# nadult/Snail

Measured on AMD Instinct MI355X. Metric: Mrays/sec (primary), higher is better.
Workload: dtype f32

## Files before the change

### snail_amd/csrc/snail_dev.inc

```
namespace SNAIL_DEV_NS {

typedef unsigned long long u64;
typedef unsigned u32x4 __attribute__((ext_vector_type(4)));
typedef const __attribute__((address_space(4))) u32x4 *scalar_ptr;

struct Node {
	float bmin[3], bmax[3];
	unsigned sub;
	int aux;
};

__device__ __forceinline__ float asf(unsigned u) { return __uint_as_float(u); }
__device__ __forceinline__ float asf(int u) { return __int_as_float(u); }

typedef const __attribute__((address_space(4))) char *scalar_bytes;
__device__ __forceinline__ Node loadNode(const uint4 *nodes, int idx) {
	const unsigned off = (unsigned)idx << 5;
	scalar_ptr p = (scalar_ptr)((scalar_bytes)(unsigned long long)nodes + off);
	u32x4 a = p[0], b = p[1];
	Node n;
	n.bmin[0] = asf(a.x); n.bmin[1] = asf(a.y); n.bmin[2] = asf(a.z);
	n.bmax[0] = asf(a.w); n.bmax[1] = asf(b.x); n.bmax[2] = asf(b.y);
	n.sub = b.z; n.aux = (int)b.w;
	return n;
// ... 627 lines not shown
		st.intersects += width;
	}
	const int q = lane - first;
#pragma unroll
	for(int l = 0; l < 4; l++) {
		const int src = (q * LPQ + l / R) * 4;
		const float d = xbar(src, ndist[l % R]);
		const int nt = __builtin_amdgcn_ds_bpermute(src, ntid[l % R]);
		if(inRange && nt >= 0) { Q.dist[l] = d; tid[l] = nt; }
	}
}
template <bool MASK, int M, bool BARY>
__device__ __forceinline__ void leafPerRay(const uint4 *__restrict__ tris, int count, int firstTri, int lane, int first, int last, const float (&org)[3][4],
										   Quad &Q, unsigned mask4, int (&tid)[4], float (&bu)[4], float (&bv)[4], Counters &st) {
	const bool inRange = lane >= first && lane <= last;
	const int width = last - first + 1;
	if(!BARY) {
		const int widthU = __builtin_amdgcn_readfirstlane(width);
		if(widthU <= 32) {
			const int firstU = __builtin_amdgcn_readfirstlane(first);
			if(widthU <= 16) leafPerRayNarrow<1, MASK, M>(tris, __builtin_amdgcn_readfirstlane(count), firstTri, lane, firstU, firstU + widthU - 1, org, Q, mask4, tid, st);
			else leafPerRayNarrow<2, MASK, M>(tris, __builtin_amdgcn_readfirstlane(count), firstTri, lane, firstU, firstU + widthU - 1, org, Q, mask4, tid, st);
			return;
		}
	}
	st.leaves++; st.fetched += (unsigned)count;
	for(int k = 0; k < count; k++) {
		const Tri t = loadTriScalar(tris, firstTri + k);
#pragma unroll
		for(int l = 0; l < 4; l++) {
			const float det = Q.d[0][l] * t.n[0] + Q.d[1][l] * t.n[1] + Q.d[2][l] * t.n[2];
			float tv[3] = {org[0][l] - t.a[0], org[1][l] - t.a[1], org[2][l] - t.a[2]};
			float c0[3] = {t.ba[1] * tv[2] - t.ba[2] * tv[1], t.ba[2] * tv[0] - t.ba[0] * tv[2], t.ba[0] * tv[1] - t.ba[1] * tv[0]};
			float c1[3] = {tv[1] * t.ca[2] - tv[2] * t.ca[1], tv[2] * t.ca[0] - tv[0] * t.ca[2], tv[0] * t.ca[1] - tv[1] * t.ca[0]};
			const float tmul = -(tv[0] * t.n[0] + tv[1] * t.n[1] + tv[2] * t.n[2]);
			const float v = (Q.d[0][l] * c0[0] + Q.d[1][l] * c0[1] + Q.d[2][l] * c0[2]) * t.it0;
			const float u = (Q.d[0][l] * c1[0] + Q.d[1][l] * c1[1] + Q.d[2][l] * c1[2]) * t.it0;
			const float duv = det - u - v;
			const float uvmin = Min3<M>(u, v, duv), uvmax = Max3<M>(u, v, duv);
			bool test = ((uvmax <= 0.0f) | (uvmin >= 0.0f)) & inRange;
			if(MASK) test = test & (((mask4 >> l) & 1u) != 0);
			if(test) {
				const float idet = Inv(det);
				const float dd = idet * tmul;
				if(dd < Q.dist[l] && dd > 0.0f) {
					Q.dist[l] = dd; tid[l] = firstTri + k;
					if(BARY) { bu[l] = u * idet; bv[l] = v * idet; }
				}
			}
		}
		st.intersects += width;
	}
}

template <bool SHARED, bool MASK, bool SHADOW, int M, bool BARY, bool DEEP, bool DISTPOS>
__device__ __forceinline__ void walk(const uint4 *__restrict__ nodes, const uint4 *__restrict__ tris, int size, int lane,
									 const float (&org)[3][4] , Quad &Q, unsigned mask4, int (&tid)[4],
									 float (&bu)[4], float (&bv)[4], float *lds, Counters &st, const int oct = 0) {
	constexpr bool EXACT = M == M_EXACT;
	Interval iv;
	{
		unsigned act4 = lane < size ? 15u : 0u;
		if(SHADOW) {
			act4 = 0;
			if(lane < size)
#pragma unroll
				for(int l = 0; l < 4; l++) act4 |= (Q.dist[l] >= 0.0f ? 1u : 0u) << l;
		} else if(MASK) act4 = lane < size ? (mask4 & 15u) : 0u;
		computeMinMax<EXACT, (MASK || SHADOW)>(Q.d, act4, size, lane, lds, iv.minDir, iv.maxDir);
		if(EXACT) computeMinMax<EXACT, (MASK || SHADOW)>(Q.id, act4, size, lane, lds, iv.minIDir, iv.maxIDir);
		else {
#pragma unroll
			for(int k = 0; k < 3; k++) iv.minIDir[k] = iv.maxIDir[k] = 0.0f;
		}
		if(SHARED) {
#pragma unroll
			for(int k = 0; k < 3; k++) iv.minOrg[k] = iv.maxOrg[k] = org[k][0];
		} else computeMinMax<EXACT, MASK>(org, act4, size, lane, lds, iv.minOrg, iv.maxOrg);
	}

	const int signBits = __builtin_amdgcn_readfirstlane((Q.d[0][0] < 0.0f ? 1 : 0) | (Q.d[1][0] < 0.0f ? 2 : 0) | (Q.d[2][0] < 0.0f ? 4 : 0));
	const int octMask[3] = {-(oct & 1), -((oct >> 1) & 1), -((oct >> 2) & 1)};

	int stkNode = 0, stkFL = 0, stkNode2 = 0, stkFL2 = 0;
	int sp = 0;
	int first = 0, last = size - 1;
	Node n = loadNode(nodes, 0);

	for(;;) {
		st.iters++;
		const bool isLeaf = (n.sub & 0x80000000u) != 0;
		const int axis = n.aux & 0xffff;
		const int firstNode = ((n.aux >> 16) ^ (signBits >> axis)) & 1;
		const int nearIdx = isLeaf ? 0 : (int)n.sub + firstNode;
		const int farIdx = (int)n.sub + (firstNode ^ 1);
		const Node nn = loadNode(nodes, nearIdx);

		auto fastPass = [&](const Node &n) -> u64 {
			float tn[4], tf[4];
			if(M == M_COH) {
				float pn[3], pf[3];
#pragma unroll
				for(int k = 0; k < 3; k++) {
					const int lo = __float_as_int(n.bmin[k]), hi = __float_as_int(n.bmax[k]);
					const int sw = (lo ^ hi) & octMask[k];
					pn[k] = __int_as_float(lo ^ sw); pf[k] = __int_as_float(hi ^ sw);
					if(SHARED) { pn[k] = pn[k] - org[k][0]; pf[k] = pf[k] - org[k][0]; }
				}
#pragma unroll
				for(int l = 0; l < 4; l++) {
					float lo[3], hi[3];
#pragma unroll
					for(int k = 0; k < 3; k++) {
						lo[k] = Q.id[k][l] * (SHARED ? pn[k] : pn[k] - org[k][l]);
						hi[k] = Q.id[k][l] * (SHARED ? pf[k] : pf[k] - org[k][l]);
					}
					tn[l] = vmax3(lo[0], lo[1], lo[2]);
					tf[l] = vmin3(hi[0], hi[1], hi[2]);
				}
			} else {
				float pn[3], pf[3];
#pragma unroll
				for(int k = 0; k < 3; k++) { pn[k] = SHARED ? n.bmin[k] - org[k][0] : n.bmin[k]; pf[k] = SHARED ? n.bmax[k] - org[k][0] : n.bmax[k]; }
#pragma unroll
				for(int l = 0; l < 4; l++) {
					float lo[3], hi[3];
#pragma unroll
					for(int k = 0; k < 3; k++) {
						const float a = Q.id[k][l] * (SHARED ? pn[k] : pn[k] - org[k][l]);
						const float b = Q.id[k][l] * (SHARED ? pf[k] : pf[k] - org[k][l]);
						lo[k] = vmin(a, b); hi[k] = vmax(a, b);
					}
					tn[l] = vmax3(lo[0], lo[1], lo[2]);
					tf[l] = vmin3(hi[0], hi[1], hi[2]);
				}
			}
			if(DISTPOS) {
#pragma unroll
				for(int l = 0; l < 4; l++) { tn[l] = vmax(tn[l], 0.0f); tf[l] = vmin(tf[l], Q.dist[l]); }
				const float slack = vmax3(tf[0] - tn[0], tf[1] - tn[1], vmax(tf[2] - tn[2], tf[3] - tn[3]));
				return __builtin_amdgcn_ballot_w64(slack >= 0.0f);
			} else {
				float sl[4];
#pragma unroll
				for(int l = 0; l < 4; l++) sl[l] = vmin(vmin(tf[l], Q.dist[l]) - tn[l], tf[l]);
				const float slack = vmax3(sl[0], sl[1], vmax(sl[2], sl[3]));
				return __builtin_amdgcn_ballot_w64(slack >= 0.0f);
			}
				};
		u64 passMask = 0;
		if(EXACT) {
			bool anyPass = false;
			if(boxTestInterval(n, iv)) {
				float tmn[3], tmx[3];
				if(SHARED) {
#pragma unroll
					for(int k = 0; k < 3; k++) { tmn[k] = n.bmin[k] - org[k][0]; tmx[k] = n.bmax[k] - org[k][0]; }
				}
#pragma unroll
				for(int l = 0; l < 4; l++) {
					float lmin = 0.0f, lmax = 0.0f;
#pragma unroll
					for(int k = 0; k < 3; k++) {
						float l1 = Q.id[k][l] * (SHARED ? tmn[k] : n.bmin[k] - org[k][l]);
						float l2 = Q.id[k][l] * (SHARED ? tmx[k] : n.bmax[k] - org[k][l]);
						float lo = Min<M_EXACT>(l1, l2), hi = Max<M_EXACT>(l1, l2);
						if(k == 0) { lmin = lo; lmax = hi; }
						else if(SHADOW) { lmin = Max<M_EXACT>(lo, lmin); lmax = Min<M_EXACT>(hi, lmax); }
						else { lmin = Max<M_EXACT>(lmin, lo); lmax = Min<M_EXACT>(lmax, hi); }
					}
					bool pass = SHADOW ? (lmax >= 0.0f && lmin <= Min<M_EXACT>(lmax, Q.dist[l])) : !(lmax < 0.0f || lmin > Min<M_EXACT>(lmax, Q.dist[l]));
					anyPass |= pass;
				}
			}
			passMask = __builtin_amdgcn_ballot_w64(anyPass);
		} else passMask = fastPass(n);
		const u64 alive = passMask & __builtin_amdgcn_ballot_w64((unsigned)(lane - first) <= (unsigned)(last - first));
		if(alive != 0) {
			first = __builtin_ctzll(alive);
			last = 63 - __builtin_clzll(alive);
			if(!isLeaf) {
				const int fl = first | (last << 8);
				if(!DEEP || sp < 64) writeLane2(stkNode, farIdx, stkFL, fl, sp);
				else writeLane2(stkNode2, farIdx, stkFL2, fl, sp - 64);
				sp++;
				n = nn;
				continue;
			}
		const int count = n.aux, firstTri = (int)(n.sub & 0x7fffffffu);
		if(SHARED) {
			if(leafShared<MASK, SHADOW, M, BARY>(tris, count, firstTri, size, lane, first, last, org, Q, mask4, tid, bu, bv, iv, st)) return;
		} else {
			leafPerRay<MASK, M, BARY>(tris, count, firstTri, lane, first, last, org, Q, mask4, tid, bu, bv, st);
		}
		}
		if(sp == 0) break;
		sp--;
		int cur, fl;
		if(!DEEP || sp < 64) { cur = __builtin_amdgcn_readlane(stkNode, sp); fl = __builtin_amdgcn_readlane(stkFL, sp); }
		else { cur = __builtin_amdgcn_readlane(stkNode2, sp - 64); fl = __builtin_amdgcn_readlane(stkFL2, sp - 64); }
		first = fl & 0xff; last = fl >> 8;
		n = loadNode(nodes, cur);
	}
}

#define SNAIL_SLAB_COH(L, NX, FX, NY, FY, NZ, FZ)                                                                                           \
	"v_mul_f32 %[t0], %[ix" L "], %[pnx]\n v_mul_f32 %[t1], %[iy" L "], %[pny]\n v_mul_f32 %[t2], %[iz" L "], %[pnz]\n"                    \
	"v_mul_f32 %[t3], %[ix" L "], %[pfx]\n v_mul_f32 %[t4], %[iy" L "], %[pfy]\n v_mul_f32 %[t5], %[iz" L "], %[pfz]\n"                    \
	"v_max3_f32 %[t0], %[t0], %[t1], %[t2]\n v_min3_f32 %[t3], %[t3], %[t4], %[t5]\n"
#define SNAIL_SLAB_FAST(L, NX, FX, NY, FY, NZ, FZ)                                                                                          \
	"v_mul_f32 %[t0], %[ix" L "], %[pnx]\n v_mul_f32 %[t3], %[ix" L "], %[pfx]\n v_min_f32 %[u0], %[t0], %[t3]\n v_max_f32 %[t3], %[t0], %[t3]\n" \
	"v_mul_f32 %[t1], %[iy" L "], %[pny]\n v_mul_f32 %[t4], %[iy" L "], %[pfy]\n v_min_f32 %[t0], %[t1], %[t4]\n v_max_f32 %[t4], %[t1], %[t4]\n" \
	"v_mul_f32 %[t2], %[iz" L "], %[pnz]\n v_mul_f32 %[t5], %[iz" L "], %[pfz]\n v_min_f32 %[t1], %[t2], %[t5]\n v_max_f32 %[t5], %[t2], %[t5]\n" \
	"v_max3_f32 %[t0], %[u0], %[t0], %[t1]\n v_min3_f32 %[t3], %[t3], %[t4], %[t5]\n"
#define SNAIL_SLAB_COH_R(L, NX, FX, NY, FY, NZ, FZ)                                                                                         \
	"v_mul_f32 %[t0], " NX ", %[ix" L "]\n v_mul_f32 %[t1], " NY ", %[iy" L "]\n v_mul_f32 %[t2], " NZ ", %[iz" L "]\n"                    \
	"v_mul_f32 %[t3], " FX ", %[ix" L "]\n v_mul_f32 %[t4], " FY ", %[iy" L "]\n v_mul_f32 %[t5], " FZ ", %[iz" L "]\n"                    \
	"v_max3_f32 %[t0], %[t0], %[t1], %[t2]\n v_min3_f32 %[t3], %[t3], %[t4], %[t5]\n"
#define SNAIL_SLAB_FAST_R(L, NX, FX, NY, FY, NZ, FZ)                                                                                        \
	"v_mul_f32 %[t0], " NX ", %[ix" L "]\n v_mul_f32 %[t3], " FX ", %[ix" L "]\n v_min_f32 %[u0], %[t0], %[t3]\n v_max_f32 %[t3], %[t0], %[t3]\n" \
	"v_mul_f32 %[t1], " NY ", %[iy" L "]\n v_mul_f32 %[t4], " FY ", %[iy" L "]\n v_min_f32 %[t0], %[t1], %[t4]\n v_max_f32 %[t4], %[t1], %[t4]\n" \
	"v_mul_f32 %[t2], " NZ ", %[iz" L "]\n v_mul_f32 %[t5], " FZ ", %[iz" L "]\n v_min_f32 %[t1], %[t2], %[t5]\n v_max_f32 %[t5], %[t2], %[t5]\n" \
	"v_max3_f32 %[t0], %[u0], %[t0], %[t1]\n v_min3_f32 %[t3], %[t3], %[t4], %[t5]\n"
#define SNAIL_SLABO_COH(L, NX, FX, NY, FY, NZ, FZ)                                                                                          \
	"v_sub_f32 %[t0], " NX ", %[ox" L "]\n v_sub_f32 %[t1], " NY ", %[oy" L "]\n v_sub_f32 %[t2], " NZ ", %[oz" L "]\n"                    \
	"v_sub_f32 %[t3], " FX ", %[ox" L "]\n v_sub_f32 %[t4], " FY ", %[oy" L "]\n v_sub_f32 %[t5], " FZ ", %[oz" L "]\n"                    \
	"v_mul_f32 %[t0], %[ix" L "], %[t0]\n v_mul_f32 %[t1], %[iy" L "], %[t1]\n v_mul_f32 %[t2], %[iz" L "], %[t2]\n"                       \
	"v_mul_f32 %[t3], %[ix" L "], %[t3]\n v_mul_f32 %[t4], %[iy" L "], %[t4]\n v_mul_f32 %[t5], %[iz" L "], %[t5]\n"                       \
	"v_max3_f32 %[t0], %[t0], %[t1], %[t2]\n v_min3_f32 %[t3], %[t3], %[t4], %[t5]\n"
#define SNAIL_SLABO_FAST(L, NX, FX, NY, FY, NZ, FZ)                                                                                         \
	"v_sub_f32 %[t0], " NX ", %[ox" L "]\n v_sub_f32 %[t3], " FX ", %[ox" L "]\n v_mul_f32 %[t0], %[ix" L "], %[t0]\n v_mul_f32 %[t3], %[ix" L "], %[t3]\n" \
	"v_min_f32 %[u0], %[t0], %[t3]\n v_max_f32 %[t3], %[t0], %[t3]\n"                                                                      \
	"v_sub_f32 %[t1], " NY ", %[oy" L "]\n v_sub_f32 %[t4], " FY ", %[oy" L "]\n v_mul_f32 %[t1], %[iy" L "], %[t1]\n v_mul_f32 %[t4], %[iy" L "], %[t4]\n" \
	"v_min_f32 %[t0], %[t1], %[t4]\n v_max_f32 %[t4], %[t1], %[t4]\n"                                                                      \
	"v_sub_f32 %[t2], " NZ ", %[oz" L "]\n v_sub_f32 %[t5], " FZ ", %[oz" L "]\n v_mul_f32 %[t2], %[iz" L "], %[t2]\n v_mul_f32 %[t5], %[iz" L "], %[t5]\n" \
	"v_min_f32 %[t1], %[t2], %[t5]\n v_max_f32 %[t5], %[t2], %[t5]\n"                                                                      \
	"v_max3_f32 %[t0], %[u0], %[t0], %[t1]\n v_min3_f32 %[t3], %[t3], %[t4], %[t5]\n"
#define SNAIL_PRE_SHARED(NX, FX, NY, FY, NZ, FZ)                                                                                            \
	" v_sub_f32 %[pnx], " NX ", %[ox]\n v_sub_f32 %[pny], " NY ", %[oy]\n v_sub_f32 %[pnz], " NZ ", %[oz]\n"                               \
	" v_sub_f32 %[pfx], " FX ", %[ox]\n v_sub_f32 %[pfy], " FY ", %[oy]\n v_sub_f32 %[pfz], " FZ ", %[oz]\n"
#define SNAIL_PRE_NONE(NX, FX, NY, FY, NZ, FZ) ""
#define SNAIL_ORG_SHARED() [ox] "v"(org[0][0]), [oy] "v"(org[1][0]), [oz] "v"(org[2][0])
#define SNAIL_ORG_PERRAY()                                                                                                                 \
	[ox0] "v"(org[0][0]), [ox1] "v"(org[0][1]), [ox2] "v"(org[0][2]), [ox3] "v"(org[0][3]), [oy0] "v"(org[1][0]), [oy1] "v"(org[1][1]),     \
		[oy2] "v"(org[1][2]), [oy3] "v"(org[1][3]), [oz0] "v"(org[2][0]), [oz1] "v"(org[2][1]), [oz2] "v"(org[2][2]), [oz3] "v"(org[2][3])
#define SNAIL_TAIL_POS(L, S) "v_max_f32 %[t0], 0, %[t0]\n v_min_f32 %[t3], %[t3], %[d" L "]\n v_sub_f32 %[" S "], %[t3], %[t0]\n"
#define SNAIL_TAIL_ANY(L, S) "v_min_f32 %[t4], %[t3], %[d" L "]\n v_sub_f32 %[t4], %[t4], %[t0]\n v_min_f32 %[" S "], %[t4], %[t3]\n"
#define SNAIL_TAIL_POSF(L, S) "v_min_f32 %[t3], %[t3], %[d" L "]\n v_sub_f32 %[" S "], %[t3], %[t0]\n"
#define SNAIL_POP_2W                                                                                                                       \
	" v_readlane_b32 %[cur], %[stkN], %[sp]\n v_readlane_b32 %[fl], %[stkF], %[sp]\n"                                                      \
	" s_and_b32 %[first], %[fl], 0xff\n s_lshr_b32 %[last], %[fl], 8\n"
#define SNAIL_PUSH_2W                                                                                                                      \
	" s_lshl_b32 %[off], %[last], 8\n s_or_b32 %[off], %[off], %[first]\n"                                                                 \
	" s_mov_b32 m0, %[sp]\n v_writelane_b32 %[stkN], %[fl], m0\n v_writelane_b32 %[stkF], %[off], m0\n"
#define SNAIL_COUNT " s_add_u32 %[cnt], %[cnt], 1\n"
#define SNAIL_DRAIN_SMEM " s_waitcnt lgkmcnt(0)\n"
#define SNAIL_DESCEND_ASM(PRE, ORGOPS, SLAB, TAIL, CNTPOP, CNTVISIT, NX, FX, NY, FY, NZ, FZ)                                                 \
	asm volatile(SNAIL_DRAIN_SMEM                                                                                                          \
				 "L_pop_%=:\n"                                                                                                             \
				 " s_cmp_eq_u32 %[sp], 0\n s_cbranch_scc1 L_done_%=\n"                                                                     \
				 " s_sub_u32 %[sp], %[sp], 1\n" CNTPOP                                                                                     \
				 SNAIL_POP_2W                                                                                                              \
				 " s_lshl_b32 %[off], %[cur], 5\n s_load_dwordx8 s[84:91], %[base], %[off]\n"                                              \
				 " s_sub_u32 %[width], %[last], %[first]\n"                                                                                \
				 " s_bfm_b64 exec, %[width], %[first]\n s_bitset1_b64 exec, %[last]\n"                                                     \
				 " s_waitcnt lgkmcnt(0)\n"                                                                                                 \
				 "L_visit_%=:\n" CNTVISIT                                                                                                  \
				 PRE(NX, FX, NY, FY, NZ, FZ)                                                                                               \
				 SLAB("0", NX, FX, NY, FY, NZ, FZ) TAIL("0", "s0") SLAB("1", NX, FX, NY, FY, NZ, FZ) TAIL("1", "s1")                       \
				 SLAB("2", NX, FX, NY, FY, NZ, FZ) TAIL("2", "s2") SLAB("3", NX, FX, NY, FY, NZ, FZ) TAIL("3", "s3")                       \
				 " v_max_f32 %[s2], %[s2], %[s3]\n v_max3_f32 %[s0], %[s0], %[s1], %[s2]\n"                                                \
				 " v_cmp_le_f32 vcc, 0, %[s0]\n"                                                                                           \
				 " s_and_b64 %[alive], vcc, exec\n s_cbranch_scc0 L_pop_%=\n"                                                              \
				 " s_ff1_i32_b64 %[first], %[alive]\n s_flbit_i32_b64 %[last], %[alive]\n s_xor_b32 %[last], %[last], 63\n"                \
				 " s_sub_u32 %[width], %[last], %[first]\n"                                                                                \
				 " s_bfm_b64 exec, %[width], %[first]\n s_bitset1_b64 exec, %[last]\n"                                                     \
				 " s_cmp_lt_i32 s90, 0\n s_cbranch_scc1 L_leaf_%=\n"                                                                       \
				 " s_lshr_b32 %[cur], %[sign16], s91\n s_xor_b32 %[cur], %[cur], s91\n s_bfe_u32 %[cur], %[cur], 0x10010\n"                \
				 " s_add_u32 %[fl], s90, 1\n s_sub_u32 %[fl], %[fl], %[cur]\n"                                                             \
				 " s_add_u32 %[cur], s90, %[cur]\n s_lshl_b32 %[off], %[cur], 5\n"                                                         \
				 " s_load_dwordx8 s[84:91], %[base], %[off]\n"                                                                             \
				 SNAIL_PUSH_2W                                                                                                             \
				 " s_add_u32 %[sp], %[sp], 1\n"                                                                                            \
				 " s_waitcnt lgkmcnt(0)\n s_branch L_visit_%=\n"                                                                           \
				 "L_leaf_%=:\n s_mov_b32 %[leafSub], s90\n s_mov_b32 %[leafAux], s91\n s_branch L_end_%=\n"                                \
				 "L_done_%=:\n s_mov_b32 %[leafSub], 0\n s_mov_b32 %[leafAux], 0\n"                                                        \
				 "L_end_%=:\n s_mov_b64 exec, -1\n"                                                                                        \
				 : [sp] "+s"(sp), [first] "+s"(first), [last] "+s"(last), [cnt] "+s"(cnt), [stkN] "+v"(stkN), [stkF] "+v"(stkF),           \
				   [leafSub] "=&s"(leafSub), [leafAux] "=&s"(leafAux), [cur] "=&s"(sCur), [fl] "=&s"(sFl), [off] "=&s"(sOff),              \
				   [width] "=&s"(sWidth), [rng] "=&s"(sRng), [alive] "=&s"(sAlive), [pnx] "=&v"(vt[0]), [pny] "=&v"(vt[1]),                \
				   [pnz] "=&v"(vt[2]), [pfx] "=&v"(vt[3]), [pfy] "=&v"(vt[4]), [pfz] "=&v"(vt[5]), [t0] "=&v"(vt[6]), [t1] "=&v"(vt[7]),   \
				   [t2] "=&v"(vt[8]), [t3] "=&v"(vt[9]), [t4] "=&v"(vt[10]), [t5] "=&v"(vt[11]), [s0] "=&v"(vt[12]), [s1] "=&v"(vt[13]),   \
				   [s2] "=&v"(vt[14]), [s3] "=&v"(vt[15]), [u0] "=&v"(vt[16])                                                              \
				 : [base] "s"(nodeBase), [sign16] "s"(sign16), [lane] "v"(lane), ORGOPS(), [ix0] "v"(Q.id[0][0]), [ix1] "v"(Q.id[0][1]), [ix2] "v"(Q.id[0][2]), [ix3] "v"(Q.id[0][3]),        \
				   [iy0] "v"(Q.id[1][0]), [iy1] "v"(Q.id[1][1]), [iy2] "v"(Q.id[1][2]), [iy3] "v"(Q.id[1][3]), [iz0] "v"(Q.id[2][0]),      \
				   [iz1] "v"(Q.id[2][1]), [iz2] "v"(Q.id[2][2]), [iz3] "v"(Q.id[2][3]), [d0] "v"(Q.dist[0]), [d1] "v"(Q.dist[1]),          \
				   [d2] "v"(Q.dist[2]), [d3] "v"(Q.dist[3])                                                                                \
				 : "s84", "s85", "s86", "s87", "s88", "s89", "s90", "s91", "vcc", "scc", "m0");                                            \
	              \
	asm volatile("" ::"s"(sp), "s"(first), "s"(last), "s"(cnt), "v"(stkN), "v"(stkF), "s"(leafSub), "s"(leafAux), "s"(sCur), "s"(sFl), "s"(sOff),    \
				 "s"(sWidth), "s"(sRng), "s"(sAlive), "v"(vt[0]), "v"(vt[1]), "v"(vt[2]), "v"(vt[3]), "v"(vt[4]), "v"(vt[5]), "v"(vt[6]), "v"(vt[7]), \
				 "v"(vt[8]), "v"(vt[9]), "v"(vt[10]), "v"(vt[11]), "v"(vt[12]), "v"(vt[13]), "v"(vt[14]), "v"(vt[15]), "v"(vt[16]))
#define SNAIL_REL_INSIDE_BIT 31
#define SNAIL_MOV_REC(D0, D1, D2, D3, S0, S1, S2, S3)                                                                                       \
	" s_mov_b64 " D0 ", " S0 "\n s_mov_b64 " D1 ", " S1 "\n s_mov_b64 " D2 ", " S2 "\n s_mov_b64 " D3 ", " S3 "\n"
#define SNAIL_A_FROM_T SNAIL_MOV_REC("s[84:85]", "s[86:87]", "s[88:89]", "s[90:91]", "s[68:69]", "s[70:71]", "s[72:73]", "s[74:75]")
#define SNAIL_PF_LEAFREQ_TRI(OTHERSET) " s_bitset0_b32 %[cur], 31\n s_load_dwordx8 " OTHERSET ", %[base], %[cur]\n"
#define SNAIL_PF_LEAFREQ_SLOT0(OTHERSET) " s_max_i32 %[cur], %[cur], 0\n s_load_dwordx8 " OTHERSET ", %[base], %[cur]\n"

#define SNAIL_PF2_NEARFAR(SUB, AUX, FARX, OTHERSET, LEAFREQ)                                                                                          \
				 " s_and_b32 %[cur], " AUX ", %[sign16]\n s_cselect_b32 %[cur], 32, 0\n"                                                       \
				 " s_xor_b32 %[cur], " SUB ", %[cur]\n s_xor_b32 " FARX ", %[cur], 32\n"                                                       \
				 LEAFREQ(OTHERSET)
#define SNAIL_PF2_TAIL(X, SUB)  \
				 " v_max_f32 %[s2], %[s2], %[s3]\n v_max3_f32 %[s0], %[s0], %[s1], %[s2]\n"                                                \
				 " v_cmpx_le_f32 vcc, 0, %[s0]\n"                                                                                           \
				 " s_cbranch_execz L_fail_%=\n"                                                                                            \
				 " s_cbranch_scc1 L_leaf" X "_%=\n"
#define SNAIL_PF2_ISLEAF(SUB) " s_cmp_lt_i32 " SUB ", 0\n"
#define SNAIL_PF2_ALIVE " s_sub_u32 %[cur], %[last], %[first]\n s_bfm_b64 %[alive], %[cur], %[first]\n s_bitset1_b64 %[alive], %[last]\n"
#define SNAIL_PF2_FIRSTLAST " s_ff1_i32_b64 %[first], exec\n s_flbit_i32_b64 %[last], exec\n s_xor_b32 %[last], %[last], 63\n"
static_assert(SNAIL_REL_INSIDE_BIT == 31, "SNAIL_OIN_TEST_SNAIL_TAIL_POS names the bit in its text");
#define SNAIL_OIN_TEST_SNAIL_TAIL_POS(AUX, CP, OMASK) " s_bitcmp1_b32 " AUX ", 31\n s_cbranch_scc1 L_oin" CP "_%=\n"
#define SNAIL_OIN_TEST_SNAIL_TAIL_ANY(AUX, CP, OMASK) ""
#define SNAIL_OIN_TEST_SNAIL_TAIL_POSF(AUX, CP, OMASK) " s_and_b32 vcc_lo, " AUX ", " OMASK "\n s_cbranch_scc0 L_slow" CP "_%=\n"
#define SNAIL_OIN_TEST_of(TAIL) SNAIL_OIN_TEST_##TAIL
#define SNAIL_OIN_PENDING(X, Y, OTHERSET, SUB, AUX, FARX, FARY, CNTVISIT, LEAFREQ)                                                          \
				 "L_oin" X "p_%=:\n" CNTVISIT                                          \
				 SNAIL_PF2_NEARFAR(SUB, AUX, FARX, OTHERSET, LEAFREQ)                                                                        \
				 SNAIL_PF2_FIRSTLAST                                                           \
				 " s_lshl_b32 %[off], %[last], 6\n s_or_b32 %[off], %[off], %[first]\n s_lshl_b32 %[off], %[off], 20\n"                    \
				 SNAIL_PF2_ALIVE                                                                                                            \
				 " s_lshr_b32 %[topw], " FARY ", 5\n s_or_b32 %[topw], %[topw], %[off]\n"                                                    \
				 " v_writelane_b32 %[stkN], %[topw], m0\n s_add_u32 m0, m0, 1\n"                                                            \
				 " s_branch L_visit" Y "p_%=\n"
#define SNAIL_OIN_COPIES_SNAIL_TAIL_POS(CNTVISIT, LEAFREQ)                                                                                  \
				 "L_oinAq_%=:\n" CNTVISIT                                                 \
				 " s_and_b32 %[cur], %[topw], 0xfffff\n s_lshl_b32 %[off], %[cur], 5\n"                                                    \
				 " s_load_dwordx8 s[68:75], %[base], %[off]\n"                                                                             \
				 SNAIL_PF2_NEARFAR("s90", "s91", "%[fl]", "s[76:83]", LEAFREQ)                                                               \
				 " s_bfe_u32 %[first], %[topw], 0x60014\n s_lshr_b32 %[last], %[topw], 26\n" SNAIL_PF2_ALIVE                               \
				 " s_branch L_visitBp_%=\n"                                                                                                \
				 SNAIL_OIN_PENDING("B", "A", "s[84:91]", "s82", "s83", "%[width]", "%[fl]", CNTVISIT, LEAFREQ)                               \
				 SNAIL_OIN_PENDING("A", "B", "s[76:83]", "s90", "s91", "%[fl]", "%[width]", CNTVISIT, LEAFREQ)
#define SNAIL_OIN_COPIES_SNAIL_TAIL_ANY(CNTVISIT, LEAFREQ) ""
#define SNAIL_OIN_COPIES_SNAIL_TAIL_POSF SNAIL_OIN_COPIES_SNAIL_TAIL_POS
#define SNAIL_OIN_COPIES_of(TAIL) SNAIL_OIN_COPIES_##TAIL
#define SNAIL_PF2_PENDING(X, OTHERSET, SUB, AUX, FARX, FARY, PRE, SLAB, TAIL, CNTVISIT, LEAFREQ, OMASK, NX, FX, NY, FY, NZ, FZ)                                            \
				 "L_visit" X "p_%=:\n"                                                                                                      \
				 " s_waitcnt lgkmcnt(0)\n"                                                 \
				 " s_load_dwordx8 s[68:75], %[base], " FARY "\n"                              \
				 SNAIL_OIN_TEST_of(TAIL)(AUX, X "p", OMASK)                                                                                   \
				 SNAIL_PF2_PENDBODY(X, OTHERSET, SUB, AUX, FARX, FARY, PRE, SLAB, TAIL, CNTVISIT, LEAFREQ, NX, FX, NY, FY, NZ, FZ)
#define SNAIL_PF2_PENDBODY(X, OTHERSET, SUB, AUX, FARX, FARY, PRE, SLAB, TAIL, CNTVISIT, LEAFREQ, NX, FX, NY, FY, NZ, FZ)                                                  \
				 CNTVISIT PRE(NX, FX, NY, FY, NZ, FZ)                                                                                        \
				 SLAB("0", NX, FX, NY, FY, NZ, FZ) TAIL("0", "s0")                                                                           \
				 SNAIL_PF2_NEARFAR(SUB, AUX, FARX, OTHERSET, LEAFREQ)                                                                        \
				 SLAB("1", NX, FX, NY, FY, NZ, FZ) TAIL("1", "s1")                                                                           \
				 SNAIL_PF2_FIRSTLAST                                                      \
				 " s_lshl_b32 %[off], %[last], 6\n s_or_b32 %[off], %[off], %[first]\n s_lshl_b32 %[off], %[off], 20\n"                    \
				 SNAIL_PF2_ALIVE                                                                                                            \
				 SLAB("2", NX, FX, NY, FY, NZ, FZ) TAIL("2", "s2")                                                                           \
				 " s_lshr_b32 %[topw], " FARY ", 5\n s_or_b32 %[topw], %[topw], %[off]\n"                                                    \
				 " v_writelane_b32 %[stkN], %[topw], m0\n s_add_u32 m0, m0, 1\n" SNAIL_PF2_ISLEAF(SUB)                                       \
				 SLAB("3", NX, FX, NY, FY, NZ, FZ) TAIL("3", "s3")                                                                           \
				 SNAIL_PF2_TAIL(X, SUB)
#define SNAIL_PF2_POPBODY(PRE, SLAB, TAIL, CNTVISIT, LEAFREQ, NXA, FXA, NYA, FYA, NZA, FZA)                                                  \
				 CNTVISIT PRE(NXA, FXA, NYA, FYA, NZA, FZA)                                                                                 \
				 SLAB("0", NXA, FXA, NYA, FYA, NZA, FZA) TAIL("0", "s0")                                                          \
				 " s_and_b32 %[cur], %[topw], 0xfffff\n s_lshl_b32 %[off], %[cur], 5\n"                                                    \
				 " s_load_dwordx8 s[68:75], %[base], %[off]\n"                                                                             \
				 SLAB("1", NXA, FXA, NYA, FYA, NZA, FZA) TAIL("1", "s1")                                                          \
				 SNAIL_PF2_NEARFAR("s90", "s91", "%[fl]", "s[76:83]", LEAFREQ)                                                                       \
				 SLAB("2", NXA, FXA, NYA, FYA, NZA, FZA) TAIL("2", "s2")                                                          \
				 " s_bfe_u32 %[first], %[topw], 0x60014\n s_lshr_b32 %[last], %[topw], 26\n" SNAIL_PF2_ALIVE SNAIL_PF2_ISLEAF("s90")        \
				 SLAB("3", NXA, FXA, NYA, FYA, NZA, FZA) TAIL("3", "s3")                                                          \
				 SNAIL_PF2_TAIL("A", "s90")
#define SNAIL_REL_NEARPOS_BIT 25
#define SNAIL_REL_FARNEG_BIT 28
#define SNAIL_REL_COUNT_MASK 0x01ffffffu
static_assert(SNAIL_REL_NEARPOS_BIT == 25 && SNAIL_REL_FARNEG_BIT == 28 && SNAIL_REL_COUNT_MASK == (1u << SNAIL_REL_NEARPOS_BIT) - 1u,
			  "SNAIL_DESCEND_PF2_OCT's masks and SNAIL_PF2_LEAF name the bits in their text");
#define SNAIL_POSENTRY_PENDING(X, Y, OTHERSET, SUB, AUX, FARX, FARY, PRE, SLAB, CNTVISIT, LEAFREQ, NX, FX, NY, FY, NZ, FZ)                    \
				 "L_slow" X "p_%=:\n"                                                   \
				 SNAIL_OIN_TEST_SNAIL_TAIL_POS(AUX, X "p", "")                                                                               \
				 SNAIL_PF2_PENDBODY(X, OTHERSET, SUB, AUX, FARX, FARY, PRE, SLAB, SNAIL_TAIL_POS, CNTVISIT, LEAFREQ, NX, FX, NY, FY, NZ, FZ)  \
				 " s_branch L_visit" Y "p_%=\n"
#define SNAIL_POSENTRY_COPIES_SNAIL_TAIL_POSF(PRE, SLAB, CNTVISIT, LEAFREQ, NXA, FXA, NYA, FYA, NZA, FZA, NXB, FXB, NYB, FYB, NZB, FZB)        \
				 "L_slowAq_%=:\n"                                                         \
				 SNAIL_OIN_TEST_SNAIL_TAIL_POS("s91", "Aq", "")                                                                              \
				 SNAIL_PF2_POPBODY(PRE, SLAB, SNAIL_TAIL_POS, CNTVISIT, LEAFREQ, NXA, FXA, NYA, FYA, NZA, FZA)                               \
				 " s_branch L_visitBp_%=\n"                                                                                                \
				 SNAIL_POSENTRY_PENDING("B", "A", "s[84:91]", "s82", "s83", "%[width]", "%[fl]", PRE, SLAB, CNTVISIT, LEAFREQ, NXB, FXB, NYB, FYB, NZB, FZB) \
				 SNAIL_POSENTRY_PENDING("A", "B", "s[76:83]", "s90", "s91", "%[fl]", "%[width]", PRE, SLAB, CNTVISIT, LEAFREQ, NXA, FXA, NYA, FYA, NZA, FZA)
#define SNAIL_POSENTRY_COPIES_SNAIL_TAIL_POS(PRE, SLAB, CNTVISIT, LEAFREQ, NXA, FXA, NYA, FYA, NZA, FZA, NXB, FXB, NYB, FYB, NZB, FZB) ""
#define SNAIL_POSENTRY_COPIES_SNAIL_TAIL_ANY(PRE, SLAB, CNTVISIT, LEAFREQ, NXA, FXA, NYA, FYA, NZA, FZA, NXB, FXB, NYB, FYB, NZB, FZB) ""
#define SNAIL_POSENTRY_COPIES_of(TAIL) SNAIL_POSENTRY_COPIES_##TAIL
#define SNAIL_PF2_LEAF(X, SUB, AUX)                                                                                                         \
				 "L_leaf" X "_%=:\n" SNAIL_PF2_FIRSTLAST                                                                                    \
				 " s_bfe_u32 %[leafSub], " SUB ", 0x190006\n s_sub_u32 %[leafSub], %[leafSub], 0x80000\n s_bitset1_b32 %[leafSub], 31\n"   \
				 " s_and_b32 %[leafAux], " AUX ", 0x01ffffff\n s_waitcnt lgkmcnt(0)\n s_branch L_end_%=\n"
#define SNAIL_DESCEND_PF2X(EXTRACLOB, OMASK, PREVARS, PRE, ORGOPS, SLAB, TAIL, CNTPOP, CNTVISIT, LEAFREQ, NXA, FXA, NYA, FYA, NZA, FZA, NXB, FXB, NYB, FYB, NZB, FZB)                                                  \
	asm volatile(SNAIL_DRAIN_SMEM " s_mov_b32 m0, %[sp]\n"                                                                                \
				 "L_entry_%=:\n"                                                                                                           \
				 " s_cmp_eq_u32 m0, 0\n s_cbranch_scc1 L_done_%=\n"                                                                     \
				 " s_sub_u32 %[off], m0, 1\n"                                                                                           \
				 " v_readlane_b32 %[topw], %[stkN], %[off]\n"                                                                              \
				 " s_and_b32 %[cur], %[topw], 0xfffff\n s_lshl_b32 %[off], %[cur], 5\n"                                                    \
				 " s_load_dwordx8 s[68:75], %[base], %[off]\n"                                                                             \
				 " s_bfe_u32 %[first], %[topw], 0x60014\n s_lshr_b32 %[last], %[topw], 26\n" SNAIL_PF2_ALIVE                               \
				 "L_pop_%=:\n"                             \
				 " s_sub_u32 m0, m0, 1\n" CNTPOP                                                                                     \
				 " s_mov_b64 exec, %[alive]\n"                                                                                             \
				 " s_waitcnt lgkmcnt(0)\n" SNAIL_A_FROM_T                                                                                  \
				                   \
				 " s_sub_u32 %[off], m0, 1\n s_max_i32 %[off], %[off], 0\n"   \
				 " v_readlane_b32 %[topw], %[stkN], %[off]\n"                                                                              \
				 SNAIL_OIN_TEST_of(TAIL)("s91", "Aq", OMASK)                                                                                 \
				 SNAIL_PF2_POPBODY(PRE, SLAB, TAIL, CNTVISIT, LEAFREQ, NXA, FXA, NYA, FYA, NZA, FZA)                                         \
				                                                                    \
				 SNAIL_PF2_PENDING("B", "s[84:91]", "s82", "s83", "%[width]", "%[fl]", PRE, SLAB, TAIL, CNTVISIT, LEAFREQ, OMASK, NXB, FXB, NYB, FYB, NZB, FZB)            \
				                                                                    \
				 SNAIL_PF2_PENDING("A", "s[76:83]", "s90", "s91", "%[fl]", "%[width]", PRE, SLAB, TAIL, CNTVISIT, LEAFREQ, OMASK, NXA, FXA, NYA, FYA, NZA, FZA)            \
				 " s_branch L_visitBp_%=\n"                                                                                                \
				 SNAIL_PF2_LEAF("A", "s90", "s91") SNAIL_PF2_LEAF("B", "s82", "s83")                                                       \
				 SNAIL_OIN_COPIES_of(TAIL)(CNTVISIT, LEAFREQ)                                                                               \
				 SNAIL_POSENTRY_COPIES_of(TAIL)(PRE, SLAB, CNTVISIT, LEAFREQ, NXA, FXA, NYA, FYA, NZA, FZA, NXB, FXB, NYB, FYB, NZB, FZB)    \
				 "L_fail_%=:\n"                                                                                                            \
				 " s_cmp_eq_u32 m0, 0\n s_cbranch_scc0 L_pop_%=\n"                                                                      \
				 "L_done_%=:\n s_mov_b32 %[leafSub], 0\n s_mov_b32 %[leafAux], 0\n s_waitcnt lgkmcnt(0)\n"                                  \
				 "L_end_%=:\n s_mov_b64 exec, -1\n s_mov_b32 %[sp], m0\n"                                                                                        \
				 : [sp] "+s"(sp), [first] "+s"(first), [last] "+s"(last), [cnt] "+s"(cnt), [stkN] "+v"(stkN), [stkF] "+v"(stkF),           \
				   [leafSub] "=&s"(leafSub), [leafAux] "=&s"(leafAux), [cur] "=&s"(sCur), [fl] "=&s"(sFl), [off] "=&s"(sOff),              \
				   [width] "=&s"(sWidth), [topw] "=&s"(sTopw), [alive] "=&s"(sAlive), PREVARS() [t0] "=&v"(vt[6]), [t1] "=&v"(vt[7]),   \
				   [t2] "=&v"(vt[8]), [t3] "=&v"(vt[9]), [t4] "=&v"(vt[10]), [t5] "=&v"(vt[11]), [s0] "=&v"(vt[12]), [s1] "=&v"(vt[13]),   \
				   [s2] "=&v"(vt[14]), [s3] "=&v"(vt[15]), [u0] "=&v"(vt[16])                                                              \
				 : [base] "s"(nodeBase), [sign16] "s"(sign16), [lane] "v"(lane), ORGOPS(), [ix0] "v"(Q.id[0][0]), [ix1] "v"(Q.id[0][1]), [ix2] "v"(Q.id[0][2]), [ix3] "v"(Q.id[0][3]),        \
				   [iy0] "v"(Q.id[1][0]), [iy1] "v"(Q.id[1][1]), [iy2] "v"(Q.id[1][2]), [iy3] "v"(Q.id[1][3]), [iz0] "v"(Q.id[2][0]),      \
				   [iz1] "v"(Q.id[2][1]), [iz2] "v"(Q.id[2][2]), [iz3] "v"(Q.id[2][3]), [d0] "v"(Q.dist[0]), [d1] "v"(Q.dist[1]),          \
				   [d2] "v"(Q.dist[2]), [d3] "v"(Q.dist[3])                                                                                \
				 : "s68", "s69", "s70", "s71", "s72", "s73", "s74", "s75", "s76", "s77", "s78", "s79", "s80", "s81", "s82", "s83", "s84", "s85", "s86", "s87", \
				   "s88", "s89", "s90", "s91", "vcc", "scc", "m0" EXTRACLOB);                                                                        \
	asm volatile("" ::"s"(sp), "s"(first), "s"(last), "s"(cnt), "v"(stkN), "v"(stkF), "s"(leafSub), "s"(leafAux), "s"(sCur), "s"(sFl), "s"(sOff),    \
				 "s"(sWidth), "s"(sTopw), "s"(sAlive), "v"(vt[6]), "v"(vt[7]), \
				 "v"(vt[8]), "v"(vt[9]), "v"(vt[10]), "v"(vt[11]), "v"(vt[12]), "v"(vt[13]), "v"(vt[14]), "v"(vt[15]), "v"(vt[16]))
#define SNAIL_PREVARS_SHARED() [pnx] "=&v"(vt[0]), [pny] "=&v"(vt[1]), [pnz] "=&v"(vt[2]), [pfx] "=&v"(vt[3]), [pfy] "=&v"(vt[4]), [pfz] "=&v"(vt[5]),
#define SNAIL_PREVARS_NONE() [pnx] "=&v"(vt[0]), [pny] "=&v"(vt[1]), [pnz] "=&v"(vt[2]), [pfx] "=&v"(vt[3]), [pfy] "=&v"(vt[4]), [pfz] "=&v"(vt[5]),
#define SNAIL_PREVARS_SNAIL_PRE_SHARED SNAIL_PREVARS_SHARED
#define SNAIL_PREVARS_SNAIL_PRE_NONE SNAIL_PREVARS_NONE
#define SNAIL_PREVARS_SNAIL_PRE_SEL SNAIL_PREVARS_NONE
#define SNAIL_PREVARS_EMPTY()
#define SNAIL_PRE_NONE_X(NX, FX, NY, FY, NZ, FZ) ""
#define SNAIL_PREVARS_SNAIL_PRE_NONE_X SNAIL_PREVARS_EMPTY
#define SNAIL_PREVARS_of(PRE) SNAIL_PREVARS_##PRE
#define SNAIL_DESCEND_PF2M(OMASK, PRE, ORGOPS, SLAB, TAIL, CNTPOP, CNTVISIT, LEAFREQ, NXA, FXA, NYA, FYA, NZA, FZA, NXB, FXB, NYB, FYB, NZB, FZB)                 \
	SNAIL_DESCEND_PF2X(, OMASK, SNAIL_PREVARS_of(PRE), PRE, ORGOPS, SLAB, TAIL, CNTPOP, CNTVISIT, LEAFREQ, NXA, FXA, NYA, FYA, NZA, FZA, NXB, FXB, NYB, FYB, NZB, FZB)
#define SNAIL_PRE_SEL(NX, FX, NY, FY, NZ, FZ)                                                                                               \
				 " s_bitcmp1_b32 %[sign16], 8\n s_cselect_b32 s62, " FX ", " NX "\n s_cselect_b32 s65, " NX ", " FX "\n"                       \
				 " s_bitcmp1_b32 %[sign16], 9\n s_cselect_b32 s63, " FY ", " NY "\n s_cselect_b32 s66, " NY ", " FY "\n"                       \
				 " s_bitcmp1_b32 %[sign16], 10\n s_cselect_b32 s64, " FZ ", " NZ "\n s_cselect_b32 s67, " NZ ", " FZ "\n"
#define SNAIL_SLABO_SEL(L, NX, FX, NY, FY, NZ, FZ) SNAIL_SLABO_COH(L, "s62", "s65", "s63", "s66", "s64", "s67")
#define SNAIL_SEL_CLOB , "s62", "s63", "s64", "s65", "s66", "s67"
#define SNAIL_DESCEND_PF2_SEL(ORGOPS, SLAB, TAIL, CNTPOP, CNTVISIT, LEAFREQ)                                                                \
	SNAIL_DESCEND_PF2X(SNAIL_SEL_CLOB, "0", SNAIL_PREVARS_NONE, SNAIL_PRE_SEL, ORGOPS, SLAB, TAIL, CNTPOP, CNTVISIT, LEAFREQ, "s84", "s87", "s85", "s88", "s86", "s89", "s76", "s79", "s77", "s80", "s78", "s81")
#define SNAIL_DESCEND_PF2_PLAIN(PRE, ORGOPS, SLAB, TAIL, CNTPOP, CNTVISIT, LEAFREQ) SNAIL_DESCEND_PF2M("0", PRE, ORGOPS, SLAB, TAIL, CNTPOP, CNTVISIT, LEAFREQ, "s84", "s87", "s85", "s88", "s86", "s89", "s76", "s79", "s77", "s80", "s78", "s81")
#define SNAIL_DESCEND_PF2_OCT(PRE, ORGOPS, SLAB, TAIL, CNTPOP, CNTVISIT, LEAFREQ, OCT)                                                                                                    \
	switch(OCT) {                                                                                                                          \
	case 0: SNAIL_DESCEND_PF2M("0x0e000000", PRE, ORGOPS, SLAB, TAIL, CNTPOP, CNTVISIT, LEAFREQ, "s84", "s87", "s85", "s88", "s86", "s89", "s76", "s79", "s77", "s80", "s78", "s81"); break;            \
	case 1: SNAIL_DESCEND_PF2M("0x1c000000", PRE, ORGOPS, SLAB, TAIL, CNTPOP, CNTVISIT, LEAFREQ, "s87", "s84", "s85", "s88", "s86", "s89", "s79", "s76", "s77", "s80", "s78", "s81"); break;            \
	case 2: SNAIL_DESCEND_PF2M("0x2a000000", PRE, ORGOPS, SLAB, TAIL, CNTPOP, CNTVISIT, LEAFREQ, "s84", "s87", "s88", "s85", "s86", "s89", "s76", "s79", "s80", "s77", "s78", "s81"); break;            \
	case 3: SNAIL_DESCEND_PF2M("0x38000000", PRE, ORGOPS, SLAB, TAIL, CNTPOP, CNTVISIT, LEAFREQ, "s87", "s84", "s88", "s85", "s86", "s89", "s79", "s76", "s80", "s77", "s78", "s81"); break;            \
	case 4: SNAIL_DESCEND_PF2M("0x46000000", PRE, ORGOPS, SLAB, TAIL, CNTPOP, CNTVISIT, LEAFREQ, "s84", "s87", "s85", "s88", "s89", "s86", "s76", "s79", "s77", "s80", "s81", "s78"); break;            \
	case 5: SNAIL_DESCEND_PF2M("0x54000000", PRE, ORGOPS, SLAB, TAIL, CNTPOP, CNTVISIT, LEAFREQ, "s87", "s84", "s85", "s88", "s89", "s86", "s79", "s76", "s77", "s80", "s81", "s78"); break;            \
	case 6: SNAIL_DESCEND_PF2M("0x62000000", PRE, ORGOPS, SLAB, TAIL, CNTPOP, CNTVISIT, LEAFREQ, "s84", "s87", "s88", "s85", "s89", "s86", "s76", "s79", "s80", "s77", "s81", "s78"); break;            \
	default: SNAIL_DESCEND_PF2M("0x70000000", PRE, ORGOPS, SLAB, TAIL, CNTPOP, CNTVISIT, LEAFREQ, "s87", "s84", "s88", "s85", "s89", "s86", "s79", "s76", "s80", "s77", "s81", "s78"); break;           \
	}

#define SNAIL_DESCEND_OCT(PRE, ORGOPS, SLAB, TAIL, CNTPOP, CNTVISIT, OCT)                                                                     \
	switch(OCT) {                                                                                                                          \
	case 0: SNAIL_DESCEND_ASM(PRE, ORGOPS, SLAB, TAIL, CNTPOP, CNTVISIT, "s84", "s87", "s85", "s88", "s86", "s89"); break;                              \
	case 1: SNAIL_DESCEND_ASM(PRE, ORGOPS, SLAB, TAIL, CNTPOP, CNTVISIT, "s87", "s84", "s85", "s88", "s86", "s89"); break;                              \
	case 2: SNAIL_DESCEND_ASM(PRE, ORGOPS, SLAB, TAIL, CNTPOP, CNTVISIT, "s84", "s87", "s88", "s85", "s86", "s89"); break;                              \
	case 3: SNAIL_DESCEND_ASM(PRE, ORGOPS, SLAB, TAIL, CNTPOP, CNTVISIT, "s87", "s84", "s88", "s85", "s86", "s89"); break;                              \
	case 4: SNAIL_DESCEND_ASM(PRE, ORGOPS, SLAB, TAIL, CNTPOP, CNTVISIT, "s84", "s87", "s85", "s88", "s89", "s86"); break;                              \
	case 5: SNAIL_DESCEND_ASM(PRE, ORGOPS, SLAB, TAIL, CNTPOP, CNTVISIT, "s87", "s84", "s85", "s88", "s89", "s86"); break;                              \
	case 6: SNAIL_DESCEND_ASM(PRE, ORGOPS, SLAB, TAIL, CNTPOP, CNTVISIT, "s84", "s87", "s88", "s85", "s89", "s86"); break;                              \
	default: SNAIL_DESCEND_ASM(PRE, ORGOPS, SLAB, TAIL, CNTPOP, CNTVISIT, "s87", "s84", "s88", "s85", "s89", "s86"); break;                             \
	}

template <bool SHADOW, bool COH, bool PACK, bool MASK, bool BARY, bool POSDIST, bool REL = true >
__device__ __forceinline__ void walkSharedAsm(const uint4 *__restrict__ nodes , const uint4 *__restrict__ tris, int size, int lane,
											  const float (&org)[3][4], Quad &Q, unsigned mask4, int (&tid)[4], float (&bu)[4], float (&bv)[4], float *lds,
											  Counters &st, const int oct) {
	Interval iv;
	{
		unsigned act4 = lane < size ? 15u : 0u;
		if(SHADOW) {
			act4 = 0;
			if(lane < size)
#pragma unroll
				for(int l = 0; l < 4; l++) act4 |= (Q.dist[l] >= 0.0f ? 1u : 0u) << l;
		} else if(MASK) act4 = lane < size ? (mask4 & 15u) : 0u;
		computeMinMax<false, (MASK || SHADOW)>(Q.d, act4, size, lane, lds, iv.minDir, iv.maxDir);
	}
#pragma unroll
	for(int k = 0; k < 3; k++) { iv.minIDir[k] = iv.maxIDir[k] = 0.0f; iv.minOrg[k] = iv.maxOrg[k] = org[k][0]; }
	const int signBits = __builtin_amdgcn_readfirstlane((Q.d[0][0] < 0.0f ? 1 : 0) | (Q.d[1][0] < 0.0f ? 2 : 0) | (Q.d[2][0] < 0.0f ? 4 : 0));
	float tidBits[4];
#pragma unroll
	for(int l = 0; l < 4; l++) tidBits[l] = __int_as_float(tid[l]);
	const int sign16 = PACK ? signBits : signBits << 16;
	const u64 nodeBase = (u64)nodes;
	float stkN = __int_as_float(PACK ? (int)((unsigned)(size - 1) << 26) | 1 : 0), stkF = __int_as_float((size - 1) << 8);
	int sp = 1, first = 0, last = size - 1, cnt = 0;
	for(;;) {
		int leafSub, leafAux, sCur, sFl, sOff, sWidth;
		u64 sRng, sAlive;
		float vt[17];
		if(PACK) {
			int sTopw;
			if(COH) {
				if(SHADOW && REL) { SNAIL_DESCEND_PF2_OCT(SNAIL_PRE_NONE_X, SNAIL_ORG_SHARED, SNAIL_SLAB_COH_R, SNAIL_TAIL_ANY, "", SNAIL_COUNT, SNAIL_PF_LEAFREQ_SLOT0, oct) }
				else if(SHADOW) { SNAIL_DESCEND_PF2_OCT(SNAIL_PRE_SHARED, SNAIL_ORG_SHARED, SNAIL_SLAB_COH, SNAIL_TAIL_ANY, "", SNAIL_COUNT, SNAIL_PF_LEAFREQ_TRI, oct) }
				else if(POSDIST) { SNAIL_DESCEND_PF2_OCT(SNAIL_PRE_NONE_X, SNAIL_ORG_SHARED, SNAIL_SLAB_COH_R, SNAIL_TAIL_POSF, SNAIL_COUNT, "", SNAIL_PF_LEAFREQ_SLOT0, oct) }
				else { SNAIL_DESCEND_PF2_OCT(SNAIL_PRE_SHARED, SNAIL_ORG_SHARED, SNAIL_SLAB_COH, SNAIL_TAIL_ANY, SNAIL_COUNT, "", SNAIL_PF_LEAFREQ_TRI, oct) }
			} else {
				if(SHADOW && REL) { SNAIL_DESCEND_PF2_PLAIN(SNAIL_PRE_NONE_X, SNAIL_ORG_SHARED, SNAIL_SLAB_FAST_R, SNAIL_TAIL_ANY, "", SNAIL_COUNT, SNAIL_PF_LEAFREQ_SLOT0); }
				else if(SHADOW) { SNAIL_DESCEND_PF2_PLAIN(SNAIL_PRE_SHARED, SNAIL_ORG_SHARED, SNAIL_SLAB_FAST, SNAIL_TAIL_ANY, "", SNAIL_COUNT, SNAIL_PF_LEAFREQ_TRI); }
				else if(POSDIST) { SNAIL_DESCEND_PF2_PLAIN(SNAIL_PRE_NONE_X, SNAIL_ORG_SHARED, SNAIL_SLAB_FAST_R, SNAIL_TAIL_POS, SNAIL_COUNT, "", SNAIL_PF_LEAFREQ_SLOT0); }
				else { SNAIL_DESCEND_PF2_PLAIN(SNAIL_PRE_SHARED, SNAIL_ORG_SHARED, SNAIL_SLAB_FAST, SNAIL_TAIL_ANY, SNAIL_COUNT, "", SNAIL_PF_LEAFREQ_TRI); }
			}
		} else if(COH) {
			if(SHADOW) { SNAIL_DESCEND_OCT(SNAIL_PRE_SHARED, SNAIL_ORG_SHARED, SNAIL_SLAB_COH, SNAIL_TAIL_ANY, "", SNAIL_COUNT, oct) }
			else if(POSDIST) { SNAIL_DESCEND_OCT(SNAIL_PRE_SHARED, SNAIL_ORG_SHARED, SNAIL_SLAB_COH, SNAIL_TAIL_POS, SNAIL_COUNT, "", oct) }
			else { SNAIL_DESCEND_OCT(SNAIL_PRE_SHARED, SNAIL_ORG_SHARED, SNAIL_SLAB_COH, SNAIL_TAIL_ANY, SNAIL_COUNT, "", oct) }
		} else {
			if(SHADOW) { SNAIL_DESCEND_ASM(SNAIL_PRE_SHARED, SNAIL_ORG_SHARED, SNAIL_SLAB_FAST, SNAIL_TAIL_ANY, "", SNAIL_COUNT, "s84", "s87", "s85", "s88", "s86", "s89"); }
			else if(POSDIST) { SNAIL_DESCEND_ASM(SNAIL_PRE_SHARED, SNAIL_ORG_SHARED, SNAIL_SLAB_FAST, SNAIL_TAIL_POS, SNAIL_COUNT, "", "s84", "s87", "s85", "s88", "s86", "s89"); }
			else { SNAIL_DESCEND_ASM(SNAIL_PRE_SHARED, SNAIL_ORG_SHARED, SNAIL_SLAB_FAST, SNAIL_TAIL_ANY, SNAIL_COUNT, "", "s84", "s87", "s85", "s88", "s86", "s89"); }
		}
		if(leafSub == 0) break;
		if(leafShared<MASK, SHADOW, COH ? M_COH : M_FAST, BARY>(tris, leafAux, (int)((unsigned)leafSub & 0x7fffffffu), size, lane, first, last, org, Q, mask4,
																 tidBits, bu, bv, iv, st))
			break;
	}
#pragma unroll
	for(int l = 0; l < 4; l++) tid[l] = __float_as_int(tidBits[l]);
	st.iters += SHADOW ? (unsigned)cnt : 2u * (unsigned)cnt - 1u;
}

template <bool MASK, bool COH, bool BARY, bool PACK>
__device__ __forceinline__ void walkPerRayAsm(const uint4 *__restrict__ nodes , const uint4 *__restrict__ tris, int size, int lane, const float (&org)[3][4],
											  Quad &Q, unsigned mask4, int (&tid)[4], float (&bu)[4], float (&bv)[4], Counters &st, const int oct) {
	const int signBits = __builtin_amdgcn_readfirstlane((Q.d[0][0] < 0.0f ? 1 : 0) | (Q.d[1][0] < 0.0f ? 2 : 0) | (Q.d[2][0] < 0.0f ? 4 : 0));
	const int sign16 = PACK ? (COH ? signBits | __builtin_amdgcn_readfirstlane(oct) << 8 : signBits) : signBits << 16;
	const u64 nodeBase = (u64)nodes;
	float stkN = __int_as_float(PACK ? (int)((unsigned)(size - 1) << 26) | 1 : 0), stkF = __int_as_float((size - 1) << 8);
	int sp = 1, first = 0, last = size - 1, cnt = 0;
	for(;;) {
		int leafSub, leafAux, sCur, sFl, sOff, sWidth;
		u64 sRng, sAlive;
		float vt[17];
		if(PACK) {
			int sTopw;
			if(COH) { SNAIL_DESCEND_PF2_SEL(SNAIL_ORG_PERRAY, SNAIL_SLABO_SEL, SNAIL_TAIL_ANY, SNAIL_COUNT, "", SNAIL_PF_LEAFREQ_TRI); }
			else { SNAIL_DESCEND_PF2_PLAIN(SNAIL_PRE_NONE, SNAIL_ORG_PERRAY, SNAIL_SLABO_FAST, SNAIL_TAIL_ANY, SNAIL_COUNT, "", SNAIL_PF_LEAFREQ_TRI); }
		} else if(COH) { SNAIL_DESCEND_OCT(SNAIL_PRE_NONE, SNAIL_ORG_PERRAY, SNAIL_SLABO_COH, SNAIL_TAIL_ANY, SNAIL_COUNT, "", oct) }
		else { SNAIL_DESCEND_ASM(SNAIL_PRE_NONE, SNAIL_ORG_PERRAY, SNAIL_SLABO_FAST, SNAIL_TAIL_ANY, SNAIL_COUNT, "", "s84", "s87", "s85", "s88", "s86", "s89"); }
		if(leafSub == 0) break;
		leafPerRay<MASK, COH ? M_COH : M_FAST, BARY>(tris, leafAux, (int)((unsigned)leafSub & 0x7fffffffu), lane, first, last, org, Q, mask4, tid, bu, bv, st);
	}
	st.iters += 2u * (unsigned)cnt - 1u;
}

__device__ __forceinline__ void finalBarycentrics(const uint4 *__restrict__ tris, const float (&org)[3][4], const Quad &Q, const int (&tid)[4],
												  float (&bu)[4], float (&bv)[4]) {
#if SNAIL_ARITH_SSE
	float det[4], uu[4], vv[4], idet[4];
#pragma unroll
	for(int l = 0; l < 4; l++) {
		det[l] = 1.0f; uu[l] = 0.0f; vv[l] = 0.0f;
		if(Q.dist[l] < __builtin_inff()) {
			const Tri t = loadTriVector(tris, tid[l]);
			const TriTerms tt = triTerms(t, org[0][0], org[1][0], org[2][0]);
			det[l] = Q.d[0][l] * t.n[0] + Q.d[1][l] * t.n[1] + Q.d[2][l] * t.n[2];
			vv[l] = Q.d[0][l] * tt.t0v[0] + Q.d[1][l] * tt.t0v[1] + Q.d[2][l] * tt.t0v[2];
			uu[l] = Q.d[0][l] * tt.t1v[0] + Q.d[1][l] * tt.t1v[1] + Q.d[2][l] * tt.t1v[2];
		}
	}
	InvN<4>(det, idet);
#pragma unroll
	for(int l = 0; l < 4; l++) {
		const bool hit = Q.dist[l] < __builtin_inff();
		bu[l] = hit ? uu[l] * idet[l] : 0.0f; bv[l] = hit ? vv[l] * idet[l] : 0.0f;
	}
#else
#pragma unroll
	for(int l = 0; l < 4; l++) {
		bu[l] = 0.0f; bv[l] = 0.0f;
		if(Q.dist[l] < __builtin_inff()) {
			const Tri t = loadTriVector(tris, tid[l]);
			const TriTerms tt = triTerms(t, org[0][0], org[1][0], org[2][0]);
			const float det = Q.d[0][l] * t.n[0] + Q.d[1][l] * t.n[1] + Q.d[2][l] * t.n[2];
			const float v = Q.d[0][l] * tt.t0v[0] + Q.d[1][l] * tt.t0v[1] + Q.d[2][l] * tt.t0v[2];
			const float u = Q.d[0][l] * tt.t1v[0] + Q.d[1][l] * tt.t1v[1] + Q.d[2][l] * tt.t1v[2];
			const float idet = Inv(det);
			bu[l] = u * idet; bv[l] = v * idet;
		}
	}
#endif
}

__device__ __forceinline__ int classify(bool fastOK, bool laneFinite, bool live, const float (&id)[3][4], const float (&dist)[4], int &oct) {
	oct = 0;
	if(!(fastOK && __all(laneFinite || !live))) return M_EXACT;
	bool coh = true;
#pragma unroll
	for(int k = 0; k < 3; k++) {
		bool anyNeg = false, anyPos = false;
#pragma unroll
		for(int l = 0; l < 4; l++) {
			const bool matters = dist[l] > -__builtin_inff();
			anyNeg |= matters && __float_as_int(id[k][l]) < 0;
			anyPos |= matters && __float_as_int(id[k][l]) >= 0;
		}
		const bool n = __any(anyNeg && live), p = __any(anyPos && live);
		coh = coh && !(n && p);
		oct |= n ? (1 << k) : 0;
	}
	return coh ? M_COH : M_FAST;
}

__device__ __forceinline__ bool originSaneDev(const float (&o)[3]) {
	return __builtin_fabsf(o[0]) <= 1.0e9f && __builtin_fabsf(o[1]) <= 1.0e9f && __builtin_fabsf(o[2]) <= 1.0e9f;
}
__device__ __forceinline__ bool finite4(const float (&v)[3][4]) {
	bool f = true;
#pragma unroll
	for(int c = 0; c < 3; c++)
#pragma unroll
		for(int l = 0; l < 4; l++) f = f && (__builtin_fabsf(v[c][l]) < __builtin_inff());
	return f;
}

__device__ __forceinline__ void flushStats(u64 *stats, const Counters &st, unsigned rays, int lane) {
	if(stats && lane == 0) {
		atomicAdd(&stats[0], (u64)st.intersects);
		atomicAdd(&stats[1], (u64)st.iters);
		atomicAdd(&stats[2], (u64)rays);
		atomicAdd(&stats[3], (u64)st.skips);
	}
}
__device__ __forceinline__ void bookPacket(unsigned *pstats, size_t packet, const Counters &st, unsigned rays, int lane) {
	if(pstats && lane == 0) {
		unsigned *w = pstats + packet * 4;
		atomicAdd(&w[0], st.intersects);
		atomicAdd(&w[1], st.iters);
		atomicAdd(&w[2], rays);
		atomicAdd(&w[3], st.skips);
	}
}

__device__ __forceinline__ int convChannelW(float c) {
	float v = c * 255.0f;
	v = v > 0.0f ? v : 0.0f;
	v = v < 255.0f ? v : 255.0f;
	return (int)v;
}

template <class ARGS>
__device__ __forceinline__ void bookPacketLate(size_t packet, const Counters &st, unsigned rays, int lane) {
	const ARGS __attribute__((address_space(4))) *E = (const ARGS __attribute__((address_space(4))) *)__builtin_amdgcn_kernarg_segment_ptr();
	asm volatile("" : "+s"(E));
	bookPacket(E->pstats, packet, st, rays, lane);
}

struct GenConst {
	float tright[3], tup[3], txyz[3][4], org[3];
};

struct FrameOut {
	float *t, *u, *v;
	int *id;
	unsigned char *bgr;
};
struct PrimaryArgs {
	const unsigned *hostTab;
	const uint4 *nodes, *tris;
	const uint4 *pf;
	int nFrames;
	GenConst g[SNAIL_MAX_BATCH];
	FrameOut out[SNAIL_MAX_BATCH];
	const uint4 *rel[SNAIL_MAX_BATCH];
	int resx, resy, x0, y0, w, h;
	const int2 *packetXY;
	int nPackets, pw, ph;
	int nBlocks;
	int pack;
	int packetMajor;
	int fastOK;
	u64 *stats;
	unsigned *cost;
	const int *order;
	int *slotCost;
	int nSlots;
	int *defer;
	int *nextOrder;
	int nextOrderFlags;
	unsigned *pstats;
};

typedef const PrimaryArgs __attribute__((address_space(4))) *PrimaryArgsK;
typedef const FrameOut __attribute__((address_space(4))) *FrameOutK;
__device__ __forceinline__ PrimaryArgsK lateArgs() {
	PrimaryArgsK p = (PrimaryArgsK)__builtin_amdgcn_kernarg_segment_ptr();
	asm volatile("" : "+s"(p));
	return p;
}

#define LDS_FLOATS_PER_WAVE (64 * 12 + 64)

__device__ __forceinline__ int interleave16(int b) {
	const int xcd = b & 7, j = b >> 3;
	return (((j >> 4) << 3) + xcd) * 16 + (j & 15);
}

template <bool DEEP, bool EXACTPASS, bool DIAG = false, bool PSTATS = false>
__device__ __forceinline__ void primaryPacket(const PrimaryArgs &A, const int li, const int fi, float *lds) {
	const int lane = threadIdx.x & 63;
	const GenConst &G = A.g[fi];

	int px, py, pidx;
	if(A.packetXY) {
		pidx = li;
		if((unsigned)pidx >= (unsigned)A.nPackets) return;
		int2 xy = A.packetXY[pidx];
		px = __builtin_amdgcn_readfirstlane(xy.x);
		py = __builtin_amdgcn_readfirstlane(xy.y);
	} else {
		const int nrx = (A.pw + 3) >> 2;
		const int region = li >> 4, k = li & 15;
		const int rx = region % nrx, ry = region / nrx;
		const int cx = rx * 4 + (k & 3), cy = ry * 4 + (k >> 2);
		if(cx >= A.pw || cy >= A.ph) {
			if(A.slotCost && fi == 0 && lane == 0 && (unsigned)li < (unsigned)A.nSlots) A.slotCost[li] = 0;
			return;
		}
		px = A.x0 + cx * 16;
		py = A.y0 + cy * 16;
		pidx = cy * A.pw + cx;
	}

	const u64 tStart = DIAG ? __builtin_amdgcn_s_memtime() : 0;
	Quad Q;
	const int ty = lane >> 2, k4 = lane & 3;
#if SNAIL_ARITH_SSE
	{
		float p[3][4], pp[4], rs[4], dn[12], idn[12];
#pragma unroll
		for(int l = 0; l < 4; l++) {
			const float xoff = (float)(px + (l >= 2 ? 2 : 0));
			const float yoff = (float)(py - (l >= 2 ? 1 : 0));
			const float tposx = (float)(4 * k4) + xoff;
			const float tposy = (float)ty + yoff;
#pragma unroll
			for(int c = 0; c < 3; c++) p[c][l] = G.tright[c] * tposx + (G.tup[c] * tposy + G.txyz[c][l]);
			pp[l] = p[0][l] * p[0][l] + p[1][l] * p[1][l] + p[2][l] * p[2][l];
		}
		RSqrtN<4>(pp, rs);
#pragma unroll
		for(int l = 0; l < 4; l++)
#pragma unroll
			for(int c = 0; c < 3; c++) { Q.d[c][l] = p[c][l] * rs[l]; dn[c * 4 + l] = Q.d[c][l] + 0.00000001f; }
		InvN<12>(dn, idn);
#pragma unroll
		for(int l = 0; l < 4; l++) {
#pragma unroll
			for(int c = 0; c < 3; c++) Q.id[c][l] = idn[c * 4 + l];
			Q.dist[l] = __builtin_inff();
		}
	}
#else
#pragma unroll
	for(int l = 0; l < 4; l++) {
		const float xoff = (float)(px + (l >= 2 ? 2 : 0));
		const float yoff = (float)(py - (l >= 2 ? 1 : 0));
		const float tposx = (float)(4 * k4) + xoff;
		const float tposy = (float)ty + yoff;
		const float p0 = G.tright[0] * tposx + (G.tup[0] * tposy + G.txyz[0][l]);
		const float p1 = G.tright[1] * tposx + (G.tup[1] * tposy + G.txyz[1][l]);
		const float p2 = G.tright[2] * tposx + (G.tup[2] * tposy + G.txyz[2][l]);
		const float rs = RSqrt(p0 * p0 + p1 * p1 + p2 * p2);
		Q.d[0][l] = p0 * rs; Q.d[1][l] = p1 * rs; Q.d[2][l] = p2 * rs;
#pragma unroll
		for(int c = 0; c < 3; c++) Q.id[c][l] = Inv(Q.d[c][l] + 0.00000001f);
		Q.dist[l] = __builtin_inff();
	}
#endif
	int tid[4] = {0, 0, 0, 0};
	float bu[4] = {0, 0, 0, 0}, bv[4] = {0, 0, 0, 0};
	float org[3][4];
#pragma unroll
	for(int c = 0; c < 3; c++)
#pragma unroll
		for(int l = 0; l < 4; l++) org[c][l] = G.org[c];

	Counters st = {0, 0, 0, 0, 0};
	int oct;
	const int mode = classify(A.fastOK != 0, finite4(Q.id) && finite4(Q.d), true, Q.id, Q.dist, oct);
	if(EXACTPASS) walk<true, false, false, M_EXACT, false, DEEP, true>(A.nodes, A.tris, 64, lane, org, Q, 15u, tid, bu, bv, lds, st);
	else if(mode == M_EXACT) {
		if(lane == 0) A.defer[2 + atomicAdd(&A.defer[0], 1)] = fi * A.nSlots + li;
		return;
	} else if(DEEP) {
		if(mode == M_COH) walk<true, false, false, M_COH, false, DEEP, true>(A.nodes, A.tris, 64, lane, org, Q, 15u, tid, bu, bv, lds, st, oct);
		else walk<true, false, false, M_FAST, false, DEEP, true>(A.nodes, A.tris, 64, lane, org, Q, 15u, tid, bu, bv, lds, st);
	} else if(A.pack && !DIAG) {
		const uint4 *pn = A.rel[fi];
		if(mode == M_COH) walkSharedAsm<false, true, true, false, false, true>(pn, A.tris, 64, lane, org, Q, 15u, tid, bu, bv, lds, st, oct);
		else walkSharedAsm<false, false, true, false, false, true>(pn, A.tris, 64, lane, org, Q, 15u, tid, bu, bv, lds, st, 0);
	} else if(mode == M_COH) walkSharedAsm<false, true, false, false, false, true>(A.nodes, A.tris, 64, lane, org, Q, 15u, tid, bu, bv, lds, st, oct);
	else walkSharedAsm<false, false, false, false, false, true>(A.nodes, A.tris, 64, lane, org, Q, 15u, tid, bu, bv, lds, st, 0);
	const PrimaryArgsK E = lateArgs();
	const FrameOutK F = &E->out[fi];
	if(F->u || F->v) finalBarycentrics(E->tris, org, Q, tid, bu, bv);

	flushStats(E->stats, st, 256u, lane);
	if(PSTATS && fi == 0) bookPacket(E->pstats, (size_t)pidx, st, 256u, lane);
	if(E->slotCost && fi == 0 && lane == 0) E->slotCost[li] = (int)st.iters;
	if(DIAG && E->cost && lane == 0) {
		const u64 tEnd = __builtin_amdgcn_s_memtime();
		unsigned *c = E->cost + (size_t)pidx * 8;
		c[0] = st.iters; c[1] = st.intersects; c[2] = (unsigned)(tEnd - tStart); c[3] = (unsigned)(tStart >> 6);
		c[4] = st.fetched; c[5] = st.leaves; c[6] = 0; c[7] = 0;
	}

	if(F->bgr) {
		unsigned bytes[12];
#pragma unroll
		for(int l = 0; l < 4; l++) {
			const float dist = InvDiv(Q.dist[l]);
			bytes[l * 3 + 0] = (unsigned)convChannelW(dist * 2.0f); bytes[l * 3 + 1] = (unsigned)convChannelW(dist * 250.0f); bytes[l * 3 + 2] = (unsigned)convChannelW(dist * 20.0f);
		}
		unsigned *o = (unsigned *)(F->bgr + ((size_t)pidx * 256 + (size_t)lane * 4) * 3);
#pragma unroll
		for(int k = 0; k < 3; k++) o[k] = bytes[4 * k] | (bytes[4 * k + 1] << 8) | (bytes[4 * k + 2] << 16) | (bytes[4 * k + 3] << 24);
	}
	if(E->packetXY || E->packetMajor) {
		const size_t o = (size_t)pidx * 256 + (size_t)lane * 4;
		if(F->t) *(float4 *)(F->t + o) = make_float4(Q.dist[0], Q.dist[1], Q.dist[2], Q.dist[3]);
		if(F->u) *(float4 *)(F->u + o) = make_float4(bu[0], bu[1], bu[2], bu[3]);
		if(F->v) *(float4 *)(F->v + o) = make_float4(bv[0], bv[1], bv[2], bv[3]);
		if(F->id) *(int4 *)(F->id + o) = make_int4(tid[0], tid[1], tid[2], tid[3]);
	} else {
		const int yy = py + ty, xx = px + k4 * 4;
		const int xlim = min(E->resx, E->x0 + E->w), ylim = min(E->resy, E->y0 + E->h);
		if(yy < ylim) {
			const size_t o = (size_t)yy * E->resx + xx;
			if(xx + 3 < xlim && (E->resx & 3) == 0) {
				if(F->t) *(float4 *)(F->t + o) = make_float4(Q.dist[0], Q.dist[1], Q.dist[2], Q.dist[3]);
// ... 1277 lines not shown
```

Before: 27930.

## Duplicate PF2 traversal state machine per mode and simplify lane-range push encoding

The packed-stack BVH descent asm is restructured so the state machine is emitted in mode-specific copies (labels suffixed per mode) that load the next node into a chosen register set, which removes the s_mov record copies between sets. The pushed lane-range encoding now stores the last-lane value straight from s_flbit (without the xor to 63), and the alive mask is rebuilt with two 64-bit shifts and an and. On push the exec mask is copied directly into alive. The initial stack word is changed to match the new encoding. This trims scalar instructions on the hot push/pop path at the cost of larger code size and instruction-cache pressure.

```diff
diff --git a/snail_amd/csrc/snail_dev.inc b/snail_amd/csrc/snail_dev.inc
--- a/snail_amd/csrc/snail_dev.inc
+++ b/snail_amd/csrc/snail_dev.inc
@@ -953,9 +953,6 @@
 				 "s"(sWidth), "s"(sRng), "s"(sAlive), "v"(vt[0]), "v"(vt[1]), "v"(vt[2]), "v"(vt[3]), "v"(vt[4]), "v"(vt[5]), "v"(vt[6]), "v"(vt[7]), \
 				 "v"(vt[8]), "v"(vt[9]), "v"(vt[10]), "v"(vt[11]), "v"(vt[12]), "v"(vt[13]), "v"(vt[14]), "v"(vt[15]), "v"(vt[16]))
 #define SNAIL_REL_INSIDE_BIT 31
-#define SNAIL_MOV_REC(D0, D1, D2, D3, S0, S1, S2, S3)                                                                                       \
-	" s_mov_b64 " D0 ", " S0 "\n s_mov_b64 " D1 ", " S1 "\n s_mov_b64 " D2 ", " S2 "\n s_mov_b64 " D3 ", " S3 "\n"
-#define SNAIL_A_FROM_T SNAIL_MOV_REC("s[84:85]", "s[86:87]", "s[88:89]", "s[90:91]", "s[68:69]", "s[70:71]", "s[72:73]", "s[74:75]")
 #define SNAIL_PF_LEAFREQ_TRI(OTHERSET) " s_bitset0_b32 %[cur], 31\n s_load_dwordx8 " OTHERSET ", %[base], %[cur]\n"
 #define SNAIL_PF_LEAFREQ_SLOT0(OTHERSET) " s_max_i32 %[cur], %[cur], 0\n s_load_dwordx8 " OTHERSET ", %[base], %[cur]\n"
 
@@ -963,122 +960,126 @@
 				 " s_and_b32 %[cur], " AUX ", %[sign16]\n s_cselect_b32 %[cur], 32, 0\n"                                                       \
 				 " s_xor_b32 %[cur], " SUB ", %[cur]\n s_xor_b32 " FARX ", %[cur], 32\n"                                                       \
 				 LEAFREQ(OTHERSET)
-#define SNAIL_PF2_TAIL(X, SUB)  \
+#define SNAIL_PF2_TAIL(X, M)  \
 				 " v_max_f32 %[s2], %[s2], %[s3]\n v_max3_f32 %[s0], %[s0], %[s1], %[s2]\n"                                                \
 				 " v_cmpx_le_f32 vcc, 0, %[s0]\n"                                                                                           \
-				 " s_cbranch_execz L_fail_%=\n"                                                                                            \
-				 " s_cbranch_scc1 L_leaf" X "_%=\n"
+				 " s_cbranch_execz L_fail" M "_%=\n"                                                                                       \
+				 " s_cbranch_scc1 L_leaf" X M "_%=\n"
 #define SNAIL_PF2_ISLEAF(SUB) " s_cmp_lt_i32 " SUB ", 0\n"
-#define SNAIL_PF2_ALIVE " s_sub_u32 %[cur], %[last], %[first]\n s_bfm_b64 %[alive], %[cur], %[first]\n s_bitset1_b64 %[alive], %[last]\n"
+#define SNAIL_PF2_ALIVE_W " s_bfe_u32 %[first], %[topw], 0x60014\n s_lshr_b32 %[last], %[topw], 26\n"                                          \
+				 " s_lshl_b64 %[alive], -1, %[first]\n s_lshr_b64 vcc, -1, %[last]\n s_and_b64 %[alive], %[alive], vcc\n"
 #define SNAIL_PF2_FIRSTLAST " s_ff1_i32_b64 %[first], exec\n s_flbit_i32_b64 %[last], exec\n s_xor_b32 %[last], %[last], 63\n"
+#define SNAIL_PF2_PUSHRANGE " s_ff1_i32_b64 %[first], exec\n s_flbit_i32_b64 %[last], exec\n"                                                  \
+				 " s_lshl_b32 %[off], %[last], 6\n s_or_b32 %[off], %[off], %[first]\n s_lshl_b32 %[off], %[off], 20\n"                    \
+				 " s_mov_b64 %[alive], exec\n"
 static_assert(SNAIL_REL_INSIDE_BIT == 31, "SNAIL_OIN_TEST_SNAIL_TAIL_POS names the bit in its text");
 #define SNAIL_OIN_TEST_SNAIL_TAIL_POS(AUX, CP, OMASK) " s_bitcmp1_b32 " AUX ", 31\n s_cbranch_scc1 L_oin" CP "_%=\n"
 #define SNAIL_OIN_TEST_SNAIL_TAIL_ANY(AUX, CP, OMASK) ""
 #define SNAIL_OIN_TEST_SNAIL_TAIL_POSF(AUX, CP, OMASK) " s_and_b32 vcc_lo, " AUX ", " OMASK "\n s_cbranch_scc0 L_slow" CP "_%=\n"
 #define SNAIL_OIN_TEST_of(TAIL) SNAIL_OIN_TEST_##TAIL
-#define SNAIL_OIN_PENDING(X, Y, OTHERSET, SUB, AUX, FARX, FARY, CNTVISIT, LEAFREQ)                                                          \
-				 "L_oin" X "p_%=:\n" CNTVISIT                                          \
+#define SNAIL_OIN_PENDING(M, X, Y, OTHERSET, SUB, AUX, FARX, FARY, CNTVISIT, LEAFREQ)                                                       \
+				 "L_oin" X "p" M "_%=:\n" CNTVISIT                                          \
 				 SNAIL_PF2_NEARFAR(SUB, AUX, FARX, OTHERSET, LEAFREQ)                                                                        \
-				 SNAIL_PF2_FIRSTLAST                                                           \
-				 " s_lshl_b32 %[off], %[last], 6\n s_or_b32 %[off], %[off], %[first]\n s_lshl_b32 %[off], %[off], 20\n"                    \
-				 SNAIL_PF2_ALIVE                                                                                                            \
+				 SNAIL_PF2_PUSHRANGE                                                           \
 				 " s_lshr_b32 %[topw], " FARY ", 5\n s_or_b32 %[topw], %[topw], %[off]\n"                                                    \
 				 " v_writelane_b32 %[stkN], %[topw], m0\n s_add_u32 m0, m0, 1\n"                                                            \
-				 " s_branch L_visit" Y "p_%=\n"
-#define SNAIL_OIN_COPIES_SNAIL_TAIL_POS(CNTVISIT, LEAFREQ)                                                                                  \
-				 "L_oinAq_%=:\n" CNTVISIT                                                 \
+				 " s_branch L_visit" Y "p" M "_%=\n"
+#define SNAIL_OIN_COPIES_SNAIL_TAIL_POS(M, XN, XSET, XSUB, XAUX, XFAR, TSET, CNTVISIT, LEAFREQ)                                             \
+				 "L_oin" XN "q" M "_%=:\n" CNTVISIT                                       \
 				 " s_and_b32 %[cur], %[topw], 0xfffff\n s_lshl_b32 %[off], %[cur], 5\n"                                                    \
-				 " s_load_dwordx8 s[68:75], %[base], %[off]\n"                                                                             \
-				 SNAIL_PF2_NEARFAR("s90", "s91", "%[fl]", "s[76:83]", LEAFREQ)                                                               \
-				 " s_bfe_u32 %[first], %[topw], 0x60014\n s_lshr_b32 %[last], %[topw], 26\n" SNAIL_PF2_ALIVE                               \
-				 " s_branch L_visitBp_%=\n"                                                                                                \
-				 SNAIL_OIN_PENDING("B", "A", "s[84:91]", "s82", "s83", "%[width]", "%[fl]", CNTVISIT, LEAFREQ)                               \
-				 SNAIL_OIN_PENDING("A", "B", "s[76:83]", "s90", "s91", "%[fl]", "%[width]", CNTVISIT, LEAFREQ)
-#define SNAIL_OIN_COPIES_SNAIL_TAIL_ANY(CNTVISIT, LEAFREQ) ""
+				 " s_load_dwordx8 " TSET ", %[base], %[off]\n"                                                                             \
+				 SNAIL_PF2_NEARFAR(XSUB, XAUX, XFAR, "s[76:83]", LEAFREQ)                                                                    \
+				 SNAIL_PF2_ALIVE_W                                                                                                          \
+				 " s_branch L_visitBp" M "_%=\n"                                                                                            \
+				 SNAIL_OIN_PENDING(M, "B", XN, XSET, "s82", "s83", "%[width]", XFAR, CNTVISIT, LEAFREQ)                                      \
+				 SNAIL_OIN_PENDING(M, XN, "B", "s[76:83]", XSUB, XAUX, XFAR, "%[width]", CNTVISIT, LEAFREQ)
+#define SNAIL_OIN_COPIES_SNAIL_TAIL_ANY(M, XN, XSET, XSUB, XAUX, XFAR, TSET, CNTVISIT, LEAFREQ) ""
 #define SNAIL_OIN_COPIES_SNAIL_TAIL_POSF SNAIL_OIN_COPIES_SNAIL_TAIL_POS
 #define SNAIL_OIN_COPIES_of(TAIL) SNAIL_OIN_COPIES_##TAIL
-#define SNAIL_PF2_PENDING(X, OTHERSET, SUB, AUX, FARX, FARY, PRE, SLAB, TAIL, CNTVISIT, LEAFREQ, OMASK, NX, FX, NY, FY, NZ, FZ)                                            \
-				 "L_visit" X "p_%=:\n"                                                                                                      \
+#define SNAIL_PF2_PENDING(M, X, TSET, OTHERSET, SUB, AUX, FARX, FARY, PRE, SLAB, TAIL, CNTVISIT, LEAFREQ, OMASK, NX, FX, NY, FY, NZ, FZ)                                            \
+				 "L_visit" X "p" M "_%=:\n"                                                                                                  \
 				 " s_waitcnt lgkmcnt(0)\n"                                                 \
-				 " s_load_dwordx8 s[68:75], %[base], " FARY "\n"                              \
-				 SNAIL_OIN_TEST_of(TAIL)(AUX, X "p", OMASK)                                                                                   \
-				 SNAIL_PF2_PENDBODY(X, OTHERSET, SUB, AUX, FARX, FARY, PRE, SLAB, TAIL, CNTVISIT, LEAFREQ, NX, FX, NY, FY, NZ, FZ)
-#define SNAIL_PF2_PENDBODY(X, OTHERSET, SUB, AUX, FARX, FARY, PRE, SLAB, TAIL, CNTVISIT, LEAFREQ, NX, FX, NY, FY, NZ, FZ)                                                  \
+				 " s_load_dwordx8 " TSET ", %[base], " FARY "\n"                              \
+				 SNAIL_OIN_TEST_of(TAIL)(AUX, X "p" M, OMASK)                                                                                 \
+				 SNAIL_PF2_PENDBODY(M, X, OTHERSET, SUB, AUX, FARX, FARY, PRE, SLAB, TAIL, CNTVISIT, LEAFREQ, NX, FX, NY, FY, NZ, FZ)
+#define SNAIL_PF2_PENDBODY(M, X, OTHERSET, SUB, AUX, FARX, FARY, PRE, SLAB, TAIL, CNTVISIT, LEAFREQ, NX, FX, NY, FY, NZ, FZ)                                                  \
 				 CNTVISIT PRE(NX, FX, NY, FY, NZ, FZ)                                                                                        \
 				 SLAB("0", NX, FX, NY, FY, NZ, FZ) TAIL("0", "s0")                                                                           \
 				 SNAIL_PF2_NEARFAR(SUB, AUX, FARX, OTHERSET, LEAFREQ)                                                                        \
 				 SLAB("1", NX, FX, NY, FY, NZ, FZ) TAIL("1", "s1")                                                                           \
-				 SNAIL_PF2_FIRSTLAST                                                      \
-				 " s_lshl_b32 %[off], %[last], 6\n s_or_b32 %[off], %[off], %[first]\n s_lshl_b32 %[off], %[off], 20\n"                    \
-				 SNAIL_PF2_ALIVE                                                                                                            \
+				 SNAIL_PF2_PUSHRANGE                                                      \
 				 SLAB("2", NX, FX, NY, FY, NZ, FZ) TAIL("2", "s2")                                                                           \
 				 " s_lshr_b32 %[topw], " FARY ", 5\n s_or_b32 %[topw], %[topw], %[off]\n"                                                    \
 				 " v_writelane_b32 %[stkN], %[topw], m0\n s_add_u32 m0, m0, 1\n" SNAIL_PF2_ISLEAF(SUB)                                       \
 				 SLAB("3", NX, FX, NY, FY, NZ, FZ) TAIL("3", "s3")                                                                           \
-				 SNAIL_PF2_TAIL(X, SUB)
-#define SNAIL_PF2_POPBODY(PRE, SLAB, TAIL, CNTVISIT, LEAFREQ, NXA, FXA, NYA, FYA, NZA, FZA)                                                  \
+				 SNAIL_PF2_TAIL(X, M)
+#define SNAIL_PF2_POPBODY(M, X, XSUB, XAUX, XFAR, TSET, PRE, SLAB, TAIL, CNTVISIT, LEAFREQ, NXA, FXA, NYA, FYA, NZA, FZA)                     \
 				 CNTVISIT PRE(NXA, FXA, NYA, FYA, NZA, FZA)                                                                                 \
 				 SLAB("0", NXA, FXA, NYA, FYA, NZA, FZA) TAIL("0", "s0")                                                          \
 				 " s_and_b32 %[cur], %[topw], 0xfffff\n s_lshl_b32 %[off], %[cur], 5\n"                                                    \
-				 " s_load_dwordx8 s[68:75], %[base], %[off]\n"                                                                             \
+				 " s_load_dwordx8 " TSET ", %[base], %[off]\n"                                                                             \
 				 SLAB("1", NXA, FXA, NYA, FYA, NZA, FZA) TAIL("1", "s1")                                                          \
-				 SNAIL_PF2_NEARFAR("s90", "s91", "%[fl]", "s[76:83]", LEAFREQ)                                                                       \
+				 SNAIL_PF2_NEARFAR(XSUB, XAUX, XFAR, "s[76:83]", LEAFREQ)                                                          \
 				 SLAB("2", NXA, FXA, NYA, FYA, NZA, FZA) TAIL("2", "s2")                                                          \
-				 " s_bfe_u32 %[first], %[topw], 0x60014\n s_lshr_b32 %[last], %[topw], 26\n" SNAIL_PF2_ALIVE SNAIL_PF2_ISLEAF("s90")        \
+				 SNAIL_PF2_ALIVE_W SNAIL_PF2_ISLEAF(XSUB)                                                                          \
 				 SLAB("3", NXA, FXA, NYA, FYA, NZA, FZA) TAIL("3", "s3")                                                          \
-				 SNAIL_PF2_TAIL("A", "s90")
+				 SNAIL_PF2_TAIL(X, M)
 #define SNAIL_REL_NEARPOS_BIT 25
 #define SNAIL_REL_FARNEG_BIT 28
 #define SNAIL_REL_COUNT_MASK 0x01ffffffu
 static_assert(SNAIL_REL_NEARPOS_BIT == 25 && SNAIL_REL_FARNEG_BIT == 28 && SNAIL_REL_COUNT_MASK == (1u << SNAIL_REL_NEARPOS_BIT) - 1u,
 			  "SNAIL_DESCEND_PF2_OCT's masks and SNAIL_PF2_LEAF name the bits in their text");
-#define SNAIL_POSENTRY_PENDING(X, Y, OTHERSET, SUB, AUX, FARX, FARY, PRE, SLAB, CNTVISIT, LEAFREQ, NX, FX, NY, FY, NZ, FZ)                    \
-				 "L_slow" X "p_%=:\n"                                                   \
-				 SNAIL_OIN_TEST_SNAIL_TAIL_POS(AUX, X "p", "")                                                                               \
-				 SNAIL_PF2_PENDBODY(X, OTHERSET, SUB, AUX, FARX, FARY, PRE, SLAB, SNAIL_TAIL_POS, CNTVISIT, LEAFREQ, NX, FX, NY, FY, NZ, FZ)  \
-				 " s_branch L_visit" Y "p_%=\n"
-#define SNAIL_POSENTRY_COPIES_SNAIL_TAIL_POSF(PRE, SLAB, CNTVISIT, LEAFREQ, NXA, FXA, NYA, FYA, NZA, FZA, NXB, FXB, NYB, FYB, NZB, FZB)        \
-				 "L_slowAq_%=:\n"                                                         \
-				 SNAIL_OIN_TEST_SNAIL_TAIL_POS("s91", "Aq", "")                                                                              \
-				 SNAIL_PF2_POPBODY(PRE, SLAB, SNAIL_TAIL_POS, CNTVISIT, LEAFREQ, NXA, FXA, NYA, FYA, NZA, FZA)                               \
-				 " s_branch L_visitBp_%=\n"                                                                                                \
-				 SNAIL_POSENTRY_PENDING("B", "A", "s[84:91]", "s82", "s83", "%[width]", "%[fl]", PRE, SLAB, CNTVISIT, LEAFREQ, NXB, FXB, NYB, FYB, NZB, FZB) \
-				 SNAIL_POSENTRY_PENDING("A", "B", "s[76:83]", "s90", "s91", "%[fl]", "%[width]", PRE, SLAB, CNTVISIT, LEAFREQ, NXA, FXA, NYA, FYA, NZA, FZA)
-#define SNAIL_POSENTRY_COPIES_SNAIL_TAIL_POS(PRE, SLAB, CNTVISIT, LEAFREQ, NXA, FXA, NYA, FYA, NZA, FZA, NXB, FXB, NYB, FYB, NZB, FZB) ""
-#define SNAIL_POSENTRY_COPIES_SNAIL_TAIL_ANY(PRE, SLAB, CNTVISIT, LEAFREQ, NXA, FXA, NYA, FYA, NZA, FZA, NXB, FXB, NYB, FYB, NZB, FZB) ""
+#define SNAIL_POSENTRY_PENDING(M, X, Y, OTHERSET, SUB, AUX, FARX, FARY, PRE, SLAB, CNTVISIT, LEAFREQ, NX, FX, NY, FY, NZ, FZ)                 \
+				 "L_slow" X "p" M "_%=:\n"                                               \
+				 SNAIL_OIN_TEST_SNAIL_TAIL_POS(AUX, X "p" M, "")                                                                             \
+				 SNAIL_PF2_PENDBODY(M, X, OTHERSET, SUB, AUX, FARX, FARY, PRE, SLAB, SNAIL_TAIL_POS, CNTVISIT, LEAFREQ, NX, FX, NY, FY, NZ, FZ) \
+				 " s_branch L_visit" Y "p" M "_%=\n"
+#define SNAIL_POSENTRY_COPIES_SNAIL_TAIL_POSF(M, XN, XSET, XSUB, XAUX, XFAR, TSET, PRE, SLAB, CNTVISIT, LEAFREQ, NXA, FXA, NYA, FYA, NZA, FZA, NXB, FXB, NYB, FYB, NZB, FZB) \
+				 "L_slow" XN "q" M "_%=:\n"                                                \
+				 SNAIL_OIN_TEST_SNAIL_TAIL_POS(XAUX, XN "q" M, "")                                                                           \
+				 SNAIL_PF2_POPBODY(M, XN, XSUB, XAUX, XFAR, TSET, PRE, SLAB, SNAIL_TAIL_POS, CNTVISIT, LEAFREQ, NXA, FXA, NYA, FYA, NZA, FZA) \
+				 " s_branch L_visitBp" M "_%=\n"                                                                                            \
+				 SNAIL_POSENTRY_PENDING(M, "B", XN, XSET, "s82", "s83", "%[width]", XFAR, PRE, SLAB, CNTVISIT, LEAFREQ, NXB, FXB, NYB, FYB, NZB, FZB) \
+				 SNAIL_POSENTRY_PENDING(M, XN, "B", "s[76:83]", XSUB, XAUX, XFAR, "%[width]", PRE, SLAB, CNTVISIT, LEAFREQ, NXA, FXA, NYA, FYA, NZA, FZA)
+#define SNAIL_POSENTRY_COPIES_SNAIL_TAIL_POS(M, XN, XSET, XSUB, XAUX, XFAR, TSET, PRE, SLAB, CNTVISIT, LEAFREQ, NXA, FXA, NYA, FYA, NZA, FZA, NXB, FXB, NYB, FYB, NZB, FZB) ""
+#define SNAIL_POSENTRY_COPIES_SNAIL_TAIL_ANY(M, XN, XSET, XSUB, XAUX, XFAR, TSET, PRE, SLAB, CNTVISIT, LEAFREQ, NXA, FXA, NYA, FYA, NZA, FZA, NXB, FXB, NYB, FYB, NZB, FZB) ""
 #define SNAIL_POSENTRY_COPIES_of(TAIL) SNAIL_POSENTRY_COPIES_##TAIL
-#define SNAIL_PF2_LEAF(X, SUB, AUX)                                                                                                         \
-				 "L_leaf" X "_%=:\n" SNAIL_PF2_FIRSTLAST                                                                                    \
+#define SNAIL_PF2_LEAF(X, M, SUB, AUX)                                                                                                      \
+				 "L_leaf" X M "_%=:\n" SNAIL_PF2_FIRSTLAST                                                                                    \
 				 " s_bfe_u32 %[leafSub], " SUB ", 0x190006\n s_sub_u32 %[leafSub], %[leafSub], 0x80000\n s_bitset1_b32 %[leafSub], 31\n"   \
 				 " s_and_b32 %[leafAux], " AUX ", 0x01ffffff\n s_waitcnt lgkmcnt(0)\n s_branch L_end_%=\n"
-#define SNAIL_DESCEND_PF2X(EXTRACLOB, OMASK, PREVARS, PRE, ORGOPS, SLAB, TAIL, CNTPOP, CNTVISIT, LEAFREQ, NXA, FXA, NYA, FYA, NZA, FZA, NXB, FXB, NYB, FYB, NZB, FZB)                                                  \
+#define SNAIL_PF2_MODE(M, OM, EMPTYBR, XN, XSET, XSUB, XAUX, XFAR, TSET, OMASK, PRE, SLAB, TAIL, CNTPOP, CNTVISIT, LEAFREQ, NXA, FXA, NYA, FYA, NZA, FZA, NXB, FXB, NYB, FYB, NZB, FZB) \
+				 "L_pop" M "_%=:\n"              \
+				 CNTPOP                                                                                                                    \
+				 " s_mov_b64 exec, %[alive]\n"                                                                                             \
+				 " s_waitcnt lgkmcnt(0)\n"              \
+				 " s_sub_u32 %[off], m0, 1\n s_max_i32 %[off], %[off], 0\n"   \
+				 " v_readlane_b32 %[topw], %[stkN], %[off]\n"                                                                              \
+				 SNAIL_OIN_TEST_of(TAIL)(XAUX, XN "q" M, OMASK)                                                                              \
+				 SNAIL_PF2_POPBODY(M, XN, XSUB, XAUX, XFAR, TSET, PRE, SLAB, TAIL, CNTVISIT, LEAFREQ, NXA, FXA, NYA, FYA, NZA, FZA)           \
+				                                                                    \
+				 SNAIL_PF2_PENDING(M, "B", TSET, XSET, "s82", "s83", "%[width]", XFAR, PRE, SLAB, TAIL, CNTVISIT, LEAFREQ, OMASK, NXB, FXB, NYB, FYB, NZB, FZB) \
+				                                                                    \
+				 SNAIL_PF2_PENDING(M, XN, TSET, "s[76:83]", XSUB, XAUX, XFAR, "%[width]", PRE, SLAB, TAIL, CNTVISIT, LEAFREQ, OMASK, NXA, FXA, NYA, FYA, NZA, FZA) \
+				 " s_branch L_visitBp" M "_%=\n"                                                                                            \
+				 SNAIL_PF2_LEAF(XN, M, XSUB, XAUX) SNAIL_PF2_LEAF("B", M, "s82", "s83")                                                      \
+				 SNAIL_OIN_COPIES_of(TAIL)(M, XN, XSET, XSUB, XAUX, XFAR, TSET, CNTVISIT, LEAFREQ)                                           \
+				 SNAIL_POSENTRY_COPIES_of(TAIL)(M, XN, XSET, XSUB, XAUX, XFAR, TSET, PRE, SLAB, CNTVISIT, LEAFREQ, NXA, FXA, NYA, FYA, NZA, FZA, NXB, FXB, NYB, FYB, NZB, FZB) \
+				 "L_fail" M "_%=:\n"                                  \
+				 " s_sub_u32 m0, m0, 1\n s_cbranch_scc0 L_pop" OM "_%=\n" EMPTYBR
+#define SNAIL_DESCEND_PF2X(EXTRACLOB, OMASK, PREVARS, PRE, ORGOPS, SLAB, TAIL, CNTPOP, CNTVISIT, LEAFREQ, NXA, FXA, NYA, FYA, NZA, FZA, NXB, FXB, NYB, FYB, NZB, FZB, NXP, FXP, NYP, FYP, NZP, FZP) \
 	asm volatile(SNAIL_DRAIN_SMEM " s_mov_b32 m0, %[sp]\n"                                                                                \
-				 "L_entry_%=:\n"                                                                                                           \
+				 "L_entry_%=:\n"     \
 				 " s_cmp_eq_u32 m0, 0\n s_cbranch_scc1 L_done_%=\n"                                                                     \
 				 " s_sub_u32 %[off], m0, 1\n"                                                                                           \
 				 " v_readlane_b32 %[topw], %[stkN], %[off]\n"                                                                              \
 				 " s_and_b32 %[cur], %[topw], 0xfffff\n s_lshl_b32 %[off], %[cur], 5\n"                                                    \
 				 " s_load_dwordx8 s[68:75], %[base], %[off]\n"                                                                             \
-				 " s_bfe_u32 %[first], %[topw], 0x60014\n s_lshr_b32 %[last], %[topw], 26\n" SNAIL_PF2_ALIVE                               \
-				 "L_pop_%=:\n"                             \
-				 " s_sub_u32 m0, m0, 1\n" CNTPOP                                                                                     \
-				 " s_mov_b64 exec, %[alive]\n"                                                                                             \
-				 " s_waitcnt lgkmcnt(0)\n" SNAIL_A_FROM_T                                                                                  \
-				                   \
-				 " s_sub_u32 %[off], m0, 1\n s_max_i32 %[off], %[off], 0\n"   \
-				 " v_readlane_b32 %[topw], %[stkN], %[off]\n"                                                                              \
-				 SNAIL_OIN_TEST_of(TAIL)("s91", "Aq", OMASK)                                                                                 \
-				 SNAIL_PF2_POPBODY(PRE, SLAB, TAIL, CNTVISIT, LEAFREQ, NXA, FXA, NYA, FYA, NZA, FZA)                                         \
-				                                                                    \
-				 SNAIL_PF2_PENDING("B", "s[84:91]", "s82", "s83", "%[width]", "%[fl]", PRE, SLAB, TAIL, CNTVISIT, LEAFREQ, OMASK, NXB, FXB, NYB, FYB, NZB, FZB)            \
-				                                                                    \
-				 SNAIL_PF2_PENDING("A", "s[76:83]", "s90", "s91", "%[fl]", "%[width]", PRE, SLAB, TAIL, CNTVISIT, LEAFREQ, OMASK, NXA, FXA, NYA, FYA, NZA, FZA)            \
-				 " s_branch L_visitBp_%=\n"                                                                                                \
-				 SNAIL_PF2_LEAF("A", "s90", "s91") SNAIL_PF2_LEAF("B", "s82", "s83")                                                       \
-				 SNAIL_OIN_COPIES_of(TAIL)(CNTVISIT, LEAFREQ)                                                                               \
-				 SNAIL_POSENTRY_COPIES_of(TAIL)(PRE, SLAB, CNTVISIT, LEAFREQ, NXA, FXA, NYA, FYA, NZA, FZA, NXB, FXB, NYB, FYB, NZB, FZB)    \
-				 "L_fail_%=:\n"                                                                                                            \
-				 " s_cmp_eq_u32 m0, 0\n s_cbranch_scc0 L_pop_%=\n"                                                                      \
+				 SNAIL_PF2_ALIVE_W                                                                                                          \
+				 " s_sub_u32 m0, m0, 1\n"                                                                                                  \
+				 SNAIL_PF2_MODE("P", "A", " s_branch L_empty_%=\n", "P", "s[68:75]", "s74", "s75", "%[leafAux]", "s[84:91]", OMASK, PRE, SLAB, TAIL, CNTPOP, CNTVISIT, LEAFREQ, NXP, FXP, NYP, FYP, NZP, FZP, NXB, FXB, NYB, FYB, NZB, FZB) \
+				 SNAIL_PF2_MODE("A", "P", "", "A", "s[84:91]", "s90", "s91", "%[fl]", "s[68:75]", OMASK, PRE, SLAB, TAIL, CNTPOP, CNTVISIT, LEAFREQ, NXA, FXA, NYA, FYA, NZA, FZA, NXB, FXB, NYB, FYB, NZB, FZB) \
+				 "L_empty_%=:\n s_mov_b32 m0, 0\n"                                                                                         \
 				 "L_done_%=:\n s_mov_b32 %[leafSub], 0\n s_mov_b32 %[leafAux], 0\n s_waitcnt lgkmcnt(0)\n"                                  \
 				 "L_end_%=:\n s_mov_b64 exec, -1\n s_mov_b32 %[sp], m0\n"                                                                                        \
 				 : [sp] "+s"(sp), [first] "+s"(first), [last] "+s"(last), [cnt] "+s"(cnt), [stkN] "+v"(stkN), [stkF] "+v"(stkF),           \
@@ -1104,8 +1105,8 @@
 #define SNAIL_PRE_NONE_X(NX, FX, NY, FY, NZ, FZ) ""
 #define SNAIL_PREVARS_SNAIL_PRE_NONE_X SNAIL_PREVARS_EMPTY
 #define SNAIL_PREVARS_of(PRE) SNAIL_PREVARS_##PRE
-#define SNAIL_DESCEND_PF2M(OMASK, PRE, ORGOPS, SLAB, TAIL, CNTPOP, CNTVISIT, LEAFREQ, NXA, FXA, NYA, FYA, NZA, FZA, NXB, FXB, NYB, FYB, NZB, FZB)                 \
-	SNAIL_DESCEND_PF2X(, OMASK, SNAIL_PREVARS_of(PRE), PRE, ORGOPS, SLAB, TAIL, CNTPOP, CNTVISIT, LEAFREQ, NXA, FXA, NYA, FYA, NZA, FZA, NXB, FXB, NYB, FYB, NZB, FZB)
+#define SNAIL_DESCEND_PF2M(OMASK, PRE, ORGOPS, SLAB, TAIL, CNTPOP, CNTVISIT, LEAFREQ, NXA, FXA, NYA, FYA, NZA, FZA, NXB, FXB, NYB, FYB, NZB, FZB, NXP, FXP, NYP, FYP, NZP, FZP) \
+	SNAIL_DESCEND_PF2X(, OMASK, SNAIL_PREVARS_of(PRE), PRE, ORGOPS, SLAB, TAIL, CNTPOP, CNTVISIT, LEAFREQ, NXA, FXA, NYA, FYA, NZA, FZA, NXB, FXB, NYB, FYB, NZB, FZB, NXP, FXP, NYP, FYP, NZP, FZP)
 #define SNAIL_PRE_SEL(NX, FX, NY, FY, NZ, FZ)                                                                                               \
 				 " s_bitcmp1_b32 %[sign16], 8\n s_cselect_b32 s62, " FX ", " NX "\n s_cselect_b32 s65, " NX ", " FX "\n"                       \
 				 " s_bitcmp1_b32 %[sign16], 9\n s_cselect_b32 s63, " FY ", " NY "\n s_cselect_b32 s66, " NY ", " FY "\n"                       \
@@ -1113,18 +1114,18 @@
 #define SNAIL_SLABO_SEL(L, NX, FX, NY, FY, NZ, FZ) SNAIL_SLABO_COH(L, "s62", "s65", "s63", "s66", "s64", "s67")
 #define SNAIL_SEL_CLOB , "s62", "s63", "s64", "s65", "s66", "s67"
 #define SNAIL_DESCEND_PF2_SEL(ORGOPS, SLAB, TAIL, CNTPOP, CNTVISIT, LEAFREQ)                                                                \
-	SNAIL_DESCEND_PF2X(SNAIL_SEL_CLOB, "0", SNAIL_PREVARS_NONE, SNAIL_PRE_SEL, ORGOPS, SLAB, TAIL, CNTPOP, CNTVISIT, LEAFREQ, "s84", "s87", "s85", "s88", "s86", "s89", "s76", "s79", "s77", "s80", "s78", "s81")
-#define SNAIL_DESCEND_PF2_PLAIN(PRE, ORGOPS, SLAB, TAIL, CNTPOP, CNTVISIT, LEAFREQ) SNAIL_DESCEND_PF2M("0", PRE, ORGOPS, SLAB, TAIL, CNTPOP, CNTVISIT, LEAFREQ, "s84", "s87", "s85", "s88", "s86", "s89", "s76", "s79", "s77", "s80", "s78", "s81")
+	SNAIL_DESCEND_PF2X(SNAIL_SEL_CLOB, "0", SNAIL_PREVARS_NONE, SNAIL_PRE_SEL, ORGOPS, SLAB, TAIL, CNTPOP, CNTVISIT, LEAFREQ, "s84", "s87", "s85", "s88", "s86", "s89", "s76", "s79", "s77", "s80", "s78", "s81", "s68", "s71", "s69", "s72", "s70", "s73")
+#define SNAIL_DESCEND_PF2_PLAIN(PRE, ORGOPS, SLAB, TAIL, CNTPOP, CNTVISIT, LEAFREQ) SNAIL_DESCEND_PF2M("0", PRE, ORGOPS, SLAB, TAIL, CNTPOP, CNTVISIT, LEAFREQ, "s84", "s87", "s85", "s88", "s86", "s89", "s76", "s79", "s77", "s80", "s78", "s81", "s68", "s71", "s69", "s72", "s70", "s73")
 #define SNAIL_DESCEND_PF2_OCT(PRE, ORGOPS, SLAB, TAIL, CNTPOP, CNTVISIT, LEAFREQ, OCT)                                                                                                    \
 	switch(OCT) {                                                                                                                          \
-	case 0: SNAIL_DESCEND_PF2M("0x0e000000", PRE, ORGOPS, SLAB, TAIL, CNTPOP, CNTVISIT, LEAFREQ, "s84", "s87", "s85", "s88", "s86", "s89", "s76", "s79", "s77", "s80", "s78", "s81"); break;            \
-	case 1: SNAIL_DESCEND_PF2M("0x1c000000", PRE, ORGOPS, SLAB, TAIL, CNTPOP, CNTVISIT, LEAFREQ, "s87", "s84", "s85", "s88", "s86", "s89", "s79", "s76", "s77", "s80", "s78", "s81"); break;            \
-	case 2: SNAIL_DESCEND_PF2M("0x2a000000", PRE, ORGOPS, SLAB, TAIL, CNTPOP, CNTVISIT, LEAFREQ, "s84", "s87", "s88", "s85", "s86", "s89", "s76", "s79", "s80", "s77", "s78", "s81"); break;            \
-	case 3: SNAIL_DESCEND_PF2M("0x38000000", PRE, ORGOPS, SLAB, TAIL, CNTPOP, CNTVISIT, LEAFREQ, "s87", "s84", "s88", "s85", "s86", "s89", "s79", "s76", "s80", "s77", "s78", "s81"); break;            \
-	case 4: SNAIL_DESCEND_PF2M("0x46000000", PRE, ORGOPS, SLAB, TAIL, CNTPOP, CNTVISIT, LEAFREQ, "s84", "s87", "s85", "s88", "s89", "s86", "s76", "s79", "s77", "s80", "s81", "s78"); break;            \
-	case 5: SNAIL_DESCEND_PF2M("0x54000000", PRE, ORGOPS, SLAB, TAIL, CNTPOP, CNTVISIT, LEAFREQ, "s87", "s84", "s85", "s88", "s89", "s86", "s79", "s76", "s77", "s80", "s81", "s78"); break;            \
-	case 6: SNAIL_DESCEND_PF2M("0x62000000", PRE, ORGOPS, SLAB, TAIL, CNTPOP, CNTVISIT, LEAFREQ, "s84", "s87", "s88", "s85", "s89", "s86", "s76", "s79", "s80", "s77", "s81", "s78"); break;            \
-	default: SNAIL_DESCEND_PF2M("0x70000000", PRE, ORGOPS, SLAB, TAIL, CNTPOP, CNTVISIT, LEAFREQ, "s87", "s84", "s88", "s85", "s89", "s86", "s79", "s76", "s80", "s77", "s81", "s78"); break;           \
+	case 0: SNAIL_DESCEND_PF2M("0x0e000000", PRE, ORGOPS, SLAB, TAIL, CNTPOP, CNTVISIT, LEAFREQ, "s84", "s87", "s85", "s88", "s86", "s89", "s76", "s79", "s77", "s80", "s78", "s81", "s68", "s71", "s69", "s72", "s70", "s73"); break;            \
+	case 1: SNAIL_DESCEND_PF2M("0x1c000000", PRE, ORGOPS, SLAB, TAIL, CNTPOP, CNTVISIT, LEAFREQ, "s87", "s84", "s85", "s88", "s86", "s89", "s79", "s76", "s77", "s80", "s78", "s81", "s71", "s68", "s69", "s72", "s70", "s73"); break;            \
+	case 2: SNAIL_DESCEND_PF2M("0x2a000000", PRE, ORGOPS, SLAB, TAIL, CNTPOP, CNTVISIT, LEAFREQ, "s84", "s87", "s88", "s85", "s86", "s89", "s76", "s79", "s80", "s77", "s78", "s81", "s68", "s71", "s72", "s69", "s70", "s73"); break;            \
+	case 3: SNAIL_DESCEND_PF2M("0x38000000", PRE, ORGOPS, SLAB, TAIL, CNTPOP, CNTVISIT, LEAFREQ, "s87", "s84", "s88", "s85", "s86", "s89", "s79", "s76", "s80", "s77", "s78", "s81", "s71", "s68", "s72", "s69", "s70", "s73"); break;            \
+	case 4: SNAIL_DESCEND_PF2M("0x46000000", PRE, ORGOPS, SLAB, TAIL, CNTPOP, CNTVISIT, LEAFREQ, "s84", "s87", "s85", "s88", "s89", "s86", "s76", "s79", "s77", "s80", "s81", "s78", "s68", "s71", "s69", "s72", "s73", "s70"); break;            \
+	case 5: SNAIL_DESCEND_PF2M("0x54000000", PRE, ORGOPS, SLAB, TAIL, CNTPOP, CNTVISIT, LEAFREQ, "s87", "s84", "s85", "s88", "s89", "s86", "s79", "s76", "s77", "s80", "s81", "s78", "s71", "s68", "s69", "s72", "s73", "s70"); break;            \
+	case 6: SNAIL_DESCEND_PF2M("0x62000000", PRE, ORGOPS, SLAB, TAIL, CNTPOP, CNTVISIT, LEAFREQ, "s84", "s87", "s88", "s85", "s89", "s86", "s76", "s79", "s80", "s77", "s81", "s78", "s68", "s71", "s72", "s69", "s73", "s70"); break;            \
+	default: SNAIL_DESCEND_PF2M("0x70000000", PRE, ORGOPS, SLAB, TAIL, CNTPOP, CNTVISIT, LEAFREQ, "s87", "s84", "s88", "s85", "s89", "s86", "s79", "s76", "s80", "s77", "s81", "s78", "s71", "s68", "s72", "s69", "s73", "s70"); break;           \
 	}
 
 #define SNAIL_DESCEND_OCT(PRE, ORGOPS, SLAB, TAIL, CNTPOP, CNTVISIT, OCT)                                                                     \
@@ -1162,7 +1163,7 @@
 	for(int l = 0; l < 4; l++) tidBits[l] = __int_as_float(tid[l]);
 	const int sign16 = PACK ? signBits : signBits << 16;
 	const u64 nodeBase = (u64)nodes;
-	float stkN = __int_as_float(PACK ? (int)((unsigned)(size - 1) << 26) | 1 : 0), stkF = __int_as_float((size - 1) << 8);
+	float stkN = __int_as_float(PACK ? (int)((unsigned)(64 - size) << 26) | 1 : 0), stkF = __int_as_float((size - 1) << 8);
 	int sp = 1, first = 0, last = size - 1, cnt = 0;
 	for(;;) {
 		int leafSub, leafAux, sCur, sFl, sOff, sWidth;
@@ -1206,7 +1207,7 @@
 	const int signBits = __builtin_amdgcn_readfirstlane((Q.d[0][0] < 0.0f ? 1 : 0) | (Q.d[1][0] < 0.0f ? 2 : 0) | (Q.d[2][0] < 0.0f ? 4 : 0));
 	const int sign16 = PACK ? (COH ? signBits | __builtin_amdgcn_readfirstlane(oct) << 8 : signBits) : signBits << 16;
 	const u64 nodeBase = (u64)nodes;
-	float stkN = __int_as_float(PACK ? (int)((unsigned)(size - 1) << 26) | 1 : 0), stkF = __int_as_float((size - 1) << 8);
+	float stkN = __int_as_float(PACK ? (int)((unsigned)(64 - size) << 26) | 1 : 0), stkF = __int_as_float((size - 1) << 8);
 	int sp = 1, first = 0, last = size - 1, cnt = 0;
 	for(;;) {
 		int leafSub, leafAux, sCur, sFl, sOff, sWidth;
```

After: 23410. 16.2% lower.
